# ufcg-lsd/custom-k8s-scheduler

Hardware: AMD Instinct MI355X
Metric: pods scheduled/sec (exact sequential stream, 5,000 nodes x 100,000 pods) (higher is better)
Workload: dtype int32+f64; 1 GPU; config2: 5,000 nodes x 100,000 pods, exact sequential, Fit+Balanced+QoS weights, percentageOfNodesToScore=100; engine=lookahead, launch=resident, table_layout=compact, lookahead=32, parallelism=single

## Files before the change

custom-k8s-scheduler_amd/csrc/qs_ctx.hpp:

```cpp
#pragma once
#include <hip/hip_runtime.h>
#include <rccl/rccl.h>

#include <mutex>
#include <string>
#include <vector>

#include "../../include/qsched.h"
#include "qs_device.hpp"
#include "qs_launch.hpp"

namespace qs_host {

constexpr int64_t kLimit = (1LL << 24) - 1;
constexpr int64_t kWideMemLimit = (1LL << 46) - 1;
constexpr int64_t kGrowLimit32 = (1LL << 31) - 1;
constexpr int64_t kGrowLimitF64 = (1LL << 53) - 1;
constexpr uint32_t kSoaMinNodes = 1u << 16;
constexpr uint32_t kAaMaxNodes = 1u << 20;

struct QsError {
    qs_status st;
    std::string msg;
};

#define HIPCHK(x)                                                                          \
    do {                                                                                   \
        hipError_t e_ = (x);                                                               \
        if (e_ != hipSuccess)                                                              \
            throw QsError{QS_EDEVICE, std::string(#x) + ": " + hipGetErrorString(e_)};     \
    } while (0)

[[noreturn]] inline void fail(qs_status st, const std::string &m) { throw QsError{st, m}; }

inline thread_local std::string g_open_err;
inline qs_status open_failed(qs_status st, const std::string &m) {
    g_open_err = m;
    return st;
}

struct DevBuf {
    void *p = nullptr;
    size_t bytes = 0;
    void ensure(size_t b) {
        if (b <= bytes) return;
        if (p) (void)hipFree(p);
        p = nullptr;
        bytes = 0;
        HIPCHK(hipMalloc(&p, b));
        bytes = b;
    }
    ~DevBuf() {
        if (p) (void)hipFree(p);
    }
    template <class T>
    T *as() const { return (T *)p; }
};

struct Mirror {
    uint32_t n = 0;
    std::vector<int64_t> ac, am, mp, rc, rm, zc, zm, np;
    std::vector<int64_t> ae, re;
    std::vector<uint64_t> th, ts, lb;
    std::vector<int32_t> zone;
    std::vector<uint64_t> gen;
    void resize(uint32_t nn) {
        n = nn;
        zone.assign(nn, 0);
        for (auto *v : {&ac, &am, &mp, &rc, &rm, &zc, &zm, &np}) v->assign(nn, 0);
        ae.assign((size_t)nn * QS_MAX_EXT, 0);
        re.assign((size_t)nn * QS_MAX_EXT, 0);
        th.assign(nn, 0);
        ts.assign(nn, 0);
        lb.assign((size_t)nn * 2, 0);
        gen.assign(nn, 0);
    }
};

inline int ctz64(int64_t v) { return v == 0 ? 64 : __builtin_ctzll((uint64_t)v); }

}

struct qs_stream {
    uint32_t p = 0;
    uint32_t feat = 0;
    std::vector<qs_pod> pods;
    std::vector<uint32_t> order;
    qs_host::DevBuf d_pods, d_podx, d_node, d_key, d_stamp;
    bool ran = false;
    int mode_ran = -1;
    uint64_t epoch_after = 0;
    int shift = 0;
    bool wide = false;
    qs_ctx *owner = nullptr;
    hipGraphExec_t gexec = nullptr;
    std::vector<uint8_t> gkey;
    ~qs_stream() {
        if (gexec) (void)hipGraphExecDestroy(gexec);
    }
};

struct qs_ctx {
    std::mutex mu;
    uint64_t table_epoch = 0;
    qs_config cfg{};
    int device = 0;
    hipStream_t stream = nullptr;
    hipStream_t stream2 = nullptr;
    std::string err;
    qs_host::Mirror m;
    int shift = 20;
    bool wide = false;
    bool dev_valid = false;
    uint32_t zero_alloc = 0;
    qs::DevTable dt{};
    qs::DevCfg dc{};
    qs_scoring_strategy strat[3] = {};
    qs_host::DevBuf strat_tab;
    std::vector<qs_stream *> streams;
    qs_host::DevBuf tbl;
    qs_host::DevBuf soa;
    bool soa_valid = false;
    qs_host::DevBuf tbl_saved;
    qs_host::Mirror m_saved;
    bool saved = false;
    bool saved_wide = false;
    int saved_shift = 20;
    bool mirror_stale = false;
    uint64_t device_faults = 0;
    qs_host::DevBuf diag;
    qs_host::DevBuf scratch, lists, clists, dio, npart, normi, nstat, nfall, nrec, bctrl, one_pod, one_podx;
    qs_host::DevBuf vshard;
    void *pin = nullptr;
    size_t pin_bytes = 0;
    uint64_t score_seq = 0;
    qs_host::DevBuf score_gs;
    uint32_t pend = 0xFFFFFFFFu;
    qs_host::DevBuf hand;
    bool handoff_off = false;
    qs_host::DevBuf resctl;
    int res_timeouts = 0;
    bool res_cooldown = false;
    uint32_t inject_used = 0;
    bool last_resident = false;
    int32_t last_res_path = 0;
    int cus = 0;
    uint64_t run_seq = 0;
    bool last_waits = false;
    uint32_t cap = 0;
    int rank = 0, world = 1;
    ncclComm_t comm = nullptr;
    qs_host::DevBuf mbox, mbox_peers;
    std::vector<void *> mbox_opened;
    bool mbox_on = false;
    bool mbox_fine = false;
    bool mbox_broken = false;
    bool mbox_host = false;
    void *mbox_hptr = nullptr;
    std::string mbox_shm;
    std::vector<void *> mbox_hmaps;
};
namespace qs_host {
void mbox_host_release(qs_ctx *c);
}

namespace qs_host {
struct ShardPlan {
    uint32_t W, v0, nv;
};
inline ShardPlan shard_plan(const qs_ctx *c) {
    if (c->world > 1) return {(uint32_t)c->world, (uint32_t)c->rank, 1u};
    if (c->cfg.virtual_shards > 1) return {(uint32_t)c->cfg.virtual_shards, 0u, (uint32_t)c->cfg.virtual_shards};
    return {1u, 0u, 1u};
}
void exchange_lists(qs_ctx *c, uint64_t *lists, size_t per_rank_entries, hipStream_t stream);
void exchange_u32(qs_ctx *c, uint32_t *buf, size_t per_rank_words, hipStream_t stream);
// ... 26 lines not shown
```

custom-k8s-scheduler_amd/csrc/qs_device.hpp:

```cpp
#pragma once
#include <hip/hip_runtime.h>
#include <hip/hip_fp16.h>
#include <stddef.h>
#include <stdint.h>

#include <type_traits>

namespace qs {

constexpr int kWave = 64;
#define QS_BAL_MAX 4

struct alignas(16) DRow {
    int32_t ac, am;
    int32_t rc, rm;
    int32_t zc, zm;
    int32_t np, mp;
    double yc, ym;
    int32_t ae0, re0, ae1, re1;
};
struct alignas(16) DRowW {
    int32_t rc, zc, np, ac;
    double rm, zm;
    double am, ym;
// ... 251 lines not shown
    constexpr int RB = (int)((F & kFeatWide) ? sizeof(DRowW) : sizeof(DRow));
    constexpr int XQ = (F & kFeatWide) ? 64 : 48;
    const u32x4 a = __builtin_amdgcn_raw_buffer_load_b128(rs, (int)i * RB, 0, 16);
    const u32x4 b = __builtin_amdgcn_raw_buffer_load_b128(rs, (int)i * RB + 16, 0, 16);
    RowT<F> r;
    if constexpr ((F & kFeatWide) != 0) {
        const int4 *q = reinterpret_cast<const int4 *>(t.wrows + i);
        const double2 c = reinterpret_cast<const double2 *>(t.wrows + i)[2];
        const int4 d = q[3];
        r.rc = (int32_t)a.x; r.zc = (int32_t)a.y; r.np = (int32_t)a.z; r.ac = (int32_t)a.w;
        r.rm = u2d(b.x, b.y); r.zm = u2d(b.z, b.w);
        r.am = c.x; r.ym = c.y;
        r.yc = u2d((uint32_t)d.x, (uint32_t)d.y);
        r.mp = d.z;
    } else {
        const double2 y = reinterpret_cast<const double2 *>(t.rows + i)[2];
        r.ac = (int32_t)a.x; r.am = (int32_t)a.y; r.rc = (int32_t)a.z; r.rm = (int32_t)a.w;
        r.zc = (int32_t)b.x; r.zm = (int32_t)b.y; r.np = (int32_t)b.z; r.mp = (int32_t)b.w;
        r.yc = y.x; r.ym = y.y;
    }
    x = RowX{};
    if (F & kFeatExt) {
        const u32x4 e = __builtin_amdgcn_raw_buffer_load_b128(rs, (int)i * RB + XQ, 0, 16);
        x.ae0 = (int32_t)e.x; x.re0 = (int32_t)e.y; x.ae1 = (int32_t)e.z; x.re1 = (int32_t)e.w;
    }
    return r;
}
template <uint32_t F>
__device__ __forceinline__ void store_row_coh(const DevTable &t, __amdgpu_buffer_rsrc_t rs, uint32_t i,
                                              const RowT<F> &r, const RowX &x) {
    (void)t;
    constexpr int RB = (int)((F & kFeatWide) ? sizeof(DRowW) : sizeof(DRow));
    constexpr int XQ = (F & kFeatWide) ? 64 : 48;
    u32x4 a, b;
    if constexpr ((F & kFeatWide) != 0) {
        const uint64_t rm = __builtin_bit_cast(uint64_t, r.rm), zm = __builtin_bit_cast(uint64_t, r.zm);
        a = u32x4{(uint32_t)r.rc, (uint32_t)r.zc, (uint32_t)r.np, (uint32_t)r.ac};
        b = u32x4{(uint32_t)rm, (uint32_t)(rm >> 32), (uint32_t)zm, (uint32_t)(zm >> 32)};
    } else {
        a = u32x4{(uint32_t)r.ac, (uint32_t)r.am, (uint32_t)r.rc, (uint32_t)r.rm};
        b = u32x4{(uint32_t)r.zc, (uint32_t)r.zm, (uint32_t)r.np, (uint32_t)r.mp};
    }
    __builtin_amdgcn_raw_buffer_store_b128(a, rs, (int)i * RB, 0, 16);
    __builtin_amdgcn_raw_buffer_store_b128(b, rs, (int)i * RB + 16, 0, 16);
    if (F & kFeatExt) {
        const u32x4 e = {(uint32_t)x.ae0, (uint32_t)x.re0, (uint32_t)x.ae1, (uint32_t)x.re1};
        __builtin_amdgcn_raw_buffer_store_b128(e, rs, (int)i * RB + XQ, 0, 16);
    }
}

struct RowQ {
    u32x4 a, b, e;
};
template <uint32_t F>
__device__ __forceinline__ RowQ load_row_q(__amdgpu_buffer_rsrc_t rs, uint32_t i) {
    static_assert((F & kFeatWide) == 0, "compact rows only");
    constexpr int kAux = 16 | (int)(1u << 31);
    RowQ q;
    q.a = __builtin_amdgcn_raw_buffer_load_b128(rs, (int)(i * sizeof(DRow)), 0, kAux);
    q.b = __builtin_amdgcn_raw_buffer_load_b128(rs, (int)(i * sizeof(DRow) + 16), 0, kAux);
    q.e = u32x4{0u, 0u, 0u, 0u};
    if (F & kFeatExt) q.e = __builtin_amdgcn_raw_buffer_load_b128(rs, (int)(i * sizeof(DRow) + 48), 0, kAux);
    return q;
}
__device__ __forceinline__ double rcp_int(int32_t a);
template <uint32_t F>
__device__ __forceinline__ Row decode_row_q(const RowQ &q, RowX &x) {
    Row r;
    r.ac = (int32_t)q.a.x; r.am = (int32_t)q.a.y; r.rc = (int32_t)q.a.z; r.rm = (int32_t)q.a.w;
    r.zc = (int32_t)q.b.x; r.zm = (int32_t)q.b.y; r.np = (int32_t)q.b.z; r.mp = (int32_t)q.b.w;
    r.yc = r.ac ? rcp_int(r.ac) : 0.0;
    r.ym = r.am ? rcp_int(r.am) : 0.0;
    x = RowX{};
    if (F & kFeatExt) { x.ae0 = (int32_t)q.e.x; x.re0 = (int32_t)q.e.y; x.ae1 = (int32_t)q.e.z; x.re1 = (int32_t)q.e.w; }
    return r;
}

template <class R, class P>
__device__ __forceinline__ void reserve(R &r, RowX &x, const P &p, int sign) {
    r.rc += sign * p.rc; r.rm += sign * p.rm;
    r.zc += sign * p.zc; r.zm += sign * p.zm;
    r.np += sign;
    x.re0 += sign * p.re0; x.re1 += sign * p.re1;
}

template <uint32_t F, class R, class P>
__device__ __forceinline__ bool fits(const R &r, const RowX &x, const P &p) {
    bool ok = r.np < r.mp;
    ok &= (p.rc <= 0) | (p.rc <= r.ac - r.rc);
    ok &= (p.rm <= 0) | (p.rm <= r.am - r.rm);
    if (F & kFeatExt) {
        ok &= (p.re0 == 0) | (p.re0 <= x.ae0 - x.re0);
        ok &= (p.re1 == 0) | (p.re1 <= x.ae1 - x.re1);
    }
    return ok;
}
__device__ __forceinline__ bool subset128(uint64_t m0, uint64_t m1, uint64_t b0, uint64_t b1) {
    return ((m0 & ~b0) | (m1 & ~b1)) == 0;
}
__device__ __forceinline__ uint64_t uniform64(uint64_t v) {
    const uint32_t lo = (uint32_t)__builtin_amdgcn_readfirstlane((int)(uint32_t)v);
    const uint32_t hi = (uint32_t)__builtin_amdgcn_readfirstlane((int)(uint32_t)(v >> 32));
    return ((uint64_t)hi << 32) | lo;
}
template <uint32_t F, class R, class P>
__device__ __forceinline__ bool feasible(const R &r, const RowX &x, const P &p, const DPodX &px) {
    bool ok = fits<F>(r, x, p);
    if (F & kFeatTaint) ok &= (x.th & ~px.tol_hard) == 0;
    if (F & kFeatAffinity) {
        const uint64_t s0 = uniform64(px.sel0), s1 = uniform64(px.sel1);
        if (s0 | s1) ok &= subset128(s0, s1, x.lb0, x.lb1);
        const uint32_t nt = (uint32_t)__builtin_amdgcn_readfirstlane((int)((p.flags >> 4) & 7u));
        if (nt != 0) {
            bool any = false;
#pragma unroll
            for (uint32_t k = 0; k < 4; ++k)
                if (k < nt) any |= subset128(px.req[k][0], px.req[k][1], x.lb0, x.lb1);
            ok &= any;
        }
    }
    return ok;
}
__device__ __forceinline__ uint32_t taint_raw(const RowX &x, const DPodX &px) {
    return (uint32_t)__popcll(x.ts & ~px.tol_soft);
}
template <class P>
__device__ __forceinline__ uint32_t affinity_raw(const RowX &x, const P &p, const DPodX &px) {
    const uint32_t nt = (uint32_t)__builtin_amdgcn_readfirstlane((int)((p.flags >> 8) & 7u));
    uint32_t s = 0;
#pragma unroll
    for (uint32_t k = 0; k < 4; ++k)
        if (k < nt) s += subset128(px.pref[k][0], px.pref[k][1], x.lb0, x.lb1) ? (uint32_t)px.pw[k] : 0u;
    return s;
}

__device__ __forceinline__ uint32_t static_raw(uint64_t th, uint64_t ts, uint64_t lb0, uint64_t lb1, uint32_t flags,
                                               const DPodX &px) {
    const uint32_t nr = (flags >> 4) & 7u, np = (flags >> 8) & 7u;
    uint32_t ok = (uint32_t)((th & ~px.tol_hard) == 0) & (uint32_t)(((px.sel0 | px.sel1) == 0) | subset128(px.sel0, px.sel1, lb0, lb1));
    uint32_t any = (uint32_t)(nr == 0), ra = 0;
#pragma unroll
    for (uint32_t k = 0; k < 4; ++k) {
        any |= (uint32_t)(k < nr) & (uint32_t)subset128(px.req[k][0], px.req[k][1], lb0, lb1);
        const uint32_t hit = (uint32_t)(k < np) & (uint32_t)subset128(px.pref[k][0], px.pref[k][1], lb0, lb1);
        ra += (0u - hit) & (uint32_t)px.pw[k];
    }
    const uint32_t rt = (uint32_t)__popcll(ts & ~px.tol_soft);
    return (ok & any) | (rt << 1) | (ra << 8);
}

__device__ __forceinline__ uint32_t floor_div(uint32_t n, double y) {
    return (uint32_t)__builtin_fma((double)n, y, 0x1p-30);
}
__device__ __forceinline__ uint32_t least_requested(int32_t a, int32_t reqd, double ya) {
    const int32_t rq = reqd < a ? reqd : a;
    const uint32_t n = __umul24((uint32_t)(a - rq), 100u);
    const uint32_t q = floor_div(n, ya);
    return reqd > a ? 0u : q;
}
__device__ __forceinline__ double fraction(int32_t a, int32_t r, double y) {
    const double R = (double)r, A = (double)a;
    const double q0 = R * y;
    const double rem = __builtin_fma(-q0, A, R);
    const double q = __builtin_fma(rem, y, q0);
    return r >= a ? 1.0 : q;
}
// ... 290 lines not shown
```

custom-k8s-scheduler_amd/csrc/qs_host.cpp:

```cpp
#include "../../include/qsched.h"

#include <hip/hip_runtime.h>

#include <algorithm>
#include <atomic>
#include <chrono>
#include <cmath>
#include <cstddef>
#include <cstdio>
#include <cstdlib>
#include <cstring>
#include <exception>
#include <mutex>
#include <new>
#include <string>
#include <vector>
#include <functional>
#include <condition_variable>
#include <thread>

#include "qs_ctx.hpp"

using namespace qs;

// ... 1233 lines not shown
        std::memset(c->pin, 0, pb);
    }
    if (!c->score_gs.p) {
        c->score_gs.ensure(32);
        HIPCHK(hipMemsetAsync(c->score_gs.p, 0, 32, c->stream));
    }
    const uint32_t pidx = c->pend < n ? c->pend : 0xFFFFFFFFu;
    const HostRow prow = pidx < n ? compact_row(c->m, pidx, c->shift, c->wide) : HostRow{};
    const uint64_t seq = ++c->score_seq;
    const auto tl = std::chrono::steady_clock::now();
    HIPCHK(launch_score_pod1(c->dt, dp, &dx, dc, static_cast<uint8_t *>(c->pin), c->score_gs.as<uint64_t>(), seq,
                             pidx, prow, c->stream));
    c->pend = 0xFFFFFFFFu;
    volatile uint64_t *done = reinterpret_cast<volatile uint64_t *>(static_cast<uint8_t *>(c->pin) + 8);
    const auto t0 = std::chrono::steady_clock::now();
    while (*done != seq) {
        if (std::chrono::steady_clock::now() - t0 > std::chrono::milliseconds(200)) {
            HIPCHK(hipStreamSynchronize(c->stream));
            if (*done != seq) fail(QS_EDEVICE, "qs_score_pod: the scoring kernel did not complete");
            break;
        }
    }
    if (g_sdiag) {
        g_split.tl = tl;
        g_split.t0 = t0;
        g_split.te = std::chrono::steady_clock::now();
    }
    std::atomic_thread_fence(std::memory_order_acquire);
    const uint8_t *h = static_cast<const uint8_t *>(c->pin);
    uint64_t kbest = 0;
    std::memcpy(&kbest, h, 8);
    if (best) *best = kbest ? (int32_t)(0xFFFFFFFFu - (uint32_t)kbest) : -1;
    return reinterpret_cast<const uint32_t *>(h + 16);
}

qs_status qs_score_pod(qs_ctx *c, const qs_pod *pod, uint8_t *feas, int32_t *score, int32_t *total,
                       int32_t *best) {
    return guarded(c, [&] {
        uint32_t w[4];
        const uint32_t *pk = score_pod_launch(c, pod, w, best);
        if (pk) unpack_scores(pk, c->m.n, w, feas, score, total);
        if (g_sdiag && pk) score_diag_report(c->score_seq, std::chrono::steady_clock::now());
    }, true);
}

qs_status qs_score_pod_packed(qs_ctx *c, const qs_pod *pod, const uint32_t **packed, int32_t *best) {
    return guarded(c, [&] {
        uint32_t w[4];
        const uint32_t *pk = score_pod_launch(c, pod, w, best);
        if (packed) *packed = pk;
        if (g_sdiag && pk) score_diag_report(c->score_seq, std::chrono::steady_clock::now());
    }, true);
}

qs_status qs_stream_prepare(qs_ctx *c, const qs_pod *pods, uint32_t p, qs_stream **out) {
    if (!out) return QS_EINVAL;
    *out = nullptr;
    qs_stream *s = nullptr;
    qs_status st = guarded(c, [&] {
        if (p && !pods) fail(QS_EINVAL, "null pods");
        HIPCHK(hipSetDevice(c->device));
        s = new qs_stream();
        s->p = p;
        s->pods.assign(pods, pods + p);
        for (uint32_t j = 0; j < p; j++) check_pod(pods[j], j);
        ensure_layout(c, pods, p);
        s->shift = c->shift;
        s->wide = c->wide;
        s->feat = feat_of(c->cfg) | (c->wide ? kFeatWide | kFeatExt : 0u);
        bool has_ext = false;
        for (uint32_t j = 0; j < p && !has_ext; j++) has_ext = pods[j].req_ext[0] || pods[j].req_ext[1];
        if (has_ext) s->feat |= kFeatExt;
        s->feat |= res_feat(c->cfg, has_ext) | strat_feat(c, pods, p);
        s->order = qos_order(pods, p, c->cfg.qos_sort != 0);
        const size_t rb = pod_record_bytes(c->wide);
        std::vector<uint8_t> dp(rb * std::max<uint32_t>(p, 1));
        const bool needx = feat_of(c->cfg) & (kFeatTaint | kFeatAffinity);
        std::vector<DPodX> dx(needx ? std::max<uint32_t>(p, 1) : 1);
        for (uint32_t k = 0; k < p; k++) {
            const uint32_t j = s->order[k];
            compact_pod(c, pods[j], j, c->shift, c->wide, dp.data() + rb * k);
            if (needx) dx[k] = compact_podx(c, pods[j]);
        }
        const size_t P1 = std::max<uint32_t>(p, 1);
        s->d_pods.ensure(rb * P1);
        s->d_podx.ensure(sizeof(DPodX) * dx.size());
        s->d_node.ensure(4 * P1);
        s->d_key.ensure(8 * P1);
        if (c->cfg.record_timestamps) s->d_stamp.ensure(8 * P1);
        HIPCHK(hipMemcpyAsync(s->d_pods.p, dp.data(), rb * p, hipMemcpyHostToDevice, c->stream));
        HIPCHK(hipMemcpyAsync(s->d_podx.p, dx.data(), sizeof(DPodX) * dx.size(), hipMemcpyHostToDevice, c->stream));
        HIPCHK(hipStreamSynchronize(c->stream));
        c->streams.push_back(s);
        s->owner = c;
    });
    if (st != QS_OK) {
        delete s;
        return st;
    }
    *out = s;
    return QS_OK;
}

qs_status qs_stream_run(qs_ctx *c, qs_stream *s, qs_mode mode, qs_stats *stats) {
    return guarded(c, [&] {
        if (!s) fail(QS_EINVAL, "null stream");
        if (mode != QS_MODE_EXACT && mode != QS_MODE_BATCHED) fail(QS_EINVAL, "unknown qs_mode");
        if (s->shift != c->shift || s->wide != c->wide) fail(QS_ESTATE, "node table re-laid out after prepare");
        HIPCHK(hipSetDevice(c->device));
        s->ran = false;
        s->mode_ran = -1;
        ++c->table_epoch;
        if (!c->dev_valid) upload_table(c);
        const uint32_t n = c->m.n, P = s->p;
        c->dc.feat = s->feat;
        const int eng = mode == QS_MODE_BATCHED ? QS_ENGINE_BATCHED : pick_engine(c, n);
        int32_t *on = s->d_node.as<int32_t>();
        uint64_t *ok = s->d_key.as<uint64_t>();
        uint64_t *st = c->cfg.record_timestamps ? s->d_stamp.as<uint64_t>() : nullptr;
        uint64_t batches = 0;
        hipEvent_t e0, e1;
        HIPCHK(hipEventCreate(&e0));
        HIPCHK(hipEventCreate(&e1));
        KernelTimer kt(c->cfg.profile_kernels != 0, c->stream, c->stream2);
        HIPCHK(hipEventRecord(e0, c->stream));
        if (P > 0 && n == 0) {
            HIPCHK(hipMemsetAsync(on, 0xFF, 4 * (size_t)P, c->stream));
            HIPCHK(hipMemsetAsync(ok, 0, 8 * (size_t)P, c->stream));
        } else if (P > 0) {
            const void *dp = s->d_pods.p;
            const DPodX *dx = s->d_podx.as<DPodX>();
            if (eng == QS_ENGINE_BATCHED) {
                batches = run_batched(c, s, dp, dx, on, ok, kt);
            } else if (eng == QS_ENGINE_PERSISTENT) {
                kt.begin(0, c->stream);
                HIPCHK(launch_persistent(c->dt, dp, dx, P, c->dc, on, ok, st, c->stream));
                kt.end(0, c->stream);
                batches = 1;
            } else if (eng == QS_ENGINE_SCAN) {
                HIPCHK(hipMemsetAsync(c->scratch.p, 0, scan_scratch_bytes(), c->stream));
                ensure_soa(c);
                for (uint32_t k = 0; k < P; k++) {
                    kt.begin(1, c->stream);
                    HIPCHK(launch_scan_pod(c->dt, dp, dx, k, c->dc, c->scratch.p, on, ok, st,
                                           nullptr, nullptr, nullptr, 1, c->stream));
                    kt.end(1, c->stream);
                    HIPCHK(launch_scan_pod(c->dt, dp, dx, k, c->dc, c->scratch.p, on, ok, st,
                                           nullptr, nullptr, nullptr, 2, c->stream));
                }
                batches = P;
            } else if (eng == QS_ENGINE_ALLREDUCE) {
                if (!c->comm)
                    fail(QS_ESTATE, "the all-reduce engine needs an RCCL communicator (qs_open_shard with an id)");
                const uint32_t V = c->world == 1 && c->cfg.virtual_shards > 1 ? (uint32_t)c->cfg.virtual_shards : 1u;
                const uint32_t R = V > 1 ? V : (uint32_t)c->world;
                DevTable dt = c->dt;
                std::memset(&dt.soa, 0, sizeof dt.soa);
                std::vector<uint32_t> sh(2 * (size_t)R);
                for (uint32_t r = 0; r < R; ++r) {
                    sh[2 * r] = (uint32_t)((uint64_t)n * r / R);
                    sh[2 * r + 1] = (uint32_t)((uint64_t)n * (r + 1) / R);
                }
                const uint32_t r0 = V > 1 ? 0u : (uint32_t)c->rank;
                c->vshard.ensure(8 * (size_t)R);
                HIPCHK(hipMemcpy(c->vshard.p, sh.data(), 8 * (size_t)R, hipMemcpyHostToDevice));
                HIPCHK(hipMemsetAsync(c->scratch.p, 0, scan_scratch_bytes(), c->stream));
                char *lohi = static_cast<char *>(c->scratch.p) + offsetof(ScanHead, lo);
                auto range = [&](uint32_t r) {
                    return hipMemcpyAsync(lohi, c->vshard.as<uint32_t>() + 2 * r, 8, hipMemcpyDeviceToDevice, c->stream);
                };
                if (V == 1) HIPCHK(range(r0));
                ScanHead *sc = c->scratch.as<ScanHead>();
                const bool norm = (c->dc.feat & (kFeatTaint | kFeatAffinity)) != 0;
                for (uint32_t k = 0; k < P; k++) {
                    kt.begin(1, c->stream);
                    if (norm) {
                        for (uint32_t v = 0; v < V; ++v) {
                            if (V > 1) HIPCHK(range(v));
                            HIPCHK(launch_scan_pod(dt, dp, dx, k, c->dc, c->scratch.p, on, ok, st, nullptr, nullptr,
                                                   nullptr, 8, c->stream));
                        }
                        allreduce_max_u32(c, &sc->mt, 2, c->stream);
                    }
                    for (uint32_t v = 0; v < V; ++v) {
                        if (V > 1) HIPCHK(range(v));
                        HIPCHK(launch_scan_pod(dt, dp, dx, k, c->dc, c->scratch.p, on, ok, st, nullptr, nullptr,
                                               nullptr, 16 | 32, c->stream));
                    }
                    allreduce_max_u64(c, reinterpret_cast<uint64_t *>(&sc->best), 1, c->stream);
                    HIPCHK(launch_scan_pod(dt, dp, dx, k, c->dc, c->scratch.p, on, ok, st, nullptr, nullptr,
                                           nullptr, 64, c->stream));
                    kt.end(1, c->stream);
                }
                batches = P;
// ... 137 lines not shown
                        }
                    }
                    hipEvent_t eend = nullptr;
                    if (handoff) {
                        HIPCHK(hipEventCreateWithFlags(&eend, hipEventDisableTiming));
                        HIPCHK(hipEventRecord(eend, c->stream2));
                        HIPCHK(hipStreamWaitEvent(c->stream, eend, 0));
                    }
                    for (int r = 0; r < R; ++r) {
                        (void)hipEventDestroy(esel[r]);
                        (void)hipEventDestroy(eres[r]);
                    }
                    (void)hipEventDestroy(est);
                    if (eend) (void)hipEventDestroy(eend);
                }
                };
                static const char *genv = getenv("QS_GRAPH");
                const bool graph_ok = !c->comm || (genv && genv[0] == '1');
                const bool use_graph = graph_ok && !handoff && !mbox && !kt.on && !diag_on && !(genv && genv[0] == '0');
                const char *renv = getenv("QS_RESIDENT");
                if (!c->cus) {
                    int cu = 0;
                    HIPCHK(hipDeviceGetAttribute(&cu, hipDeviceAttributeMultiprocessorCount, c->device));
                    c->cus = cu;
                }
                LaGeom pgeo = geo;
                if (norm && overlap && !(nw && nw[0] == '1')) pgeo.waves = 4;
                const char *rk = getenv("QS_RES_K32");
                if (rk && rk[0] == '0') pgeo.k32 = 0;
                LaGeom rgeo = la_stream_res_plan(pgeo, c->dc.feat, n, (uint32_t)c->cus, 2);
                if (rgeo.G > 0 && rgeo.K * rgeo.G + 1 > la_stream_res_max_blocks(rgeo, c->dc.feat, n, (uint32_t)c->cus))
                    rgeo = la_stream_res_plan(pgeo, c->dc.feat, n, (uint32_t)c->cus, 1);
                static const char *senv = getenv("QS_RES_SEL");
                uint32_t sel = rgeo.K * rgeo.G;
                if (senv && atoi(senv) > 0) sel = (uint32_t)atoi(senv);
                if (norm) sel = std::max(sel, rgeo.K * rgeo.G);
                const bool coresident =
                    rgeo.G > 0 && 1 + sel <= la_stream_res_max_blocks(rgeo, c->dc.feat, n, (uint32_t)c->cus);
                const bool res_transport = c->world == 1 ? !mbox && !c->comm : mbox;
                const bool res_allowed = c->res_timeouts < 2 && !c->res_cooldown;
                const bool resident = overlap && res_transport && res_allowed && !diag_on &&
                                      !(renv && renv[0] == '0') && rgeo.G > 0 && coresident;
                c->last_resident = resident;
                if (!resident) c->res_cooldown = false;
                if (resident) {
                    c->resctl.ensure(la_stream_res_ctl_bytes());
                    c->dc.ready = nullptr;
                    c->dc.epoch = 0;
                    c->dc.werr = reinterpret_cast<uint32_t *>(hw + 2);
                    c->last_waits = true;
                    HIPCHK(hipMemsetAsync(c->lists.p, 0, 8 * lwords * nbuf, c->stream));
                    HIPCHK(hipMemsetAsync(c->dio.p, 0, 2 * kDioWords * 4, c->stream));
                    HIPCHK(hipMemsetAsync(c->resctl.p, 0, la_stream_res_ctl_bytes(), c->stream));
                    HIPCHK(hipMemsetAsync(hw + 2, 0, 8, c->stream));
                    c->npart.ensure(16 * 2 * (size_t)rgeo.K * rgeo.G);
                    c->normi.ensure(16 * 2 * 64);
                    c->nstat.ensure(4 * 2 * 128 * (size_t)rgeo.K);
                    HIPCHK(hipMemsetAsync(c->nfall.p, 0, 16, c->stream));
                    const size_t rcw = std::max<size_t>(1, (size_t)rgeo.K * rgeo.G * rgeo.L);
                    c->clists.ensure(8 * rcw * 2);
                    ResShard rsh{1u, 0u, 0ull, nullptr, 0ull, 0ull, 0ull, 0ull, 0ull};
                    if (c->world > 1)
                        rsh = ResShard{(uint32_t)c->world, (uint32_t)c->rank, seq_run, c->mbox_peers.as<char *>(),
                                       kMbResHello, kMbResFlags, kMbResLists, kMbResNFlags, kMbResNorm};
                    DevCfg dcr = c->dc;
                    const char *inj = getenv("QS_INJECT_FAULT");
                    dcr.inject = (inject_once(c, "resident_stall", kInjResidentStall) ||
                                  (inj && std::strcmp(inj, "resident_stall_always") == 0)) ? 1u : 0u;
                    if (inj && std::strcmp(inj, "resident_skew") == 0) dcr.inject = 2u;
                    dcr.first_ticks = c->world > 1 ? 500000000ull : 0ull;
                    const char *fa = getenv("QS_FAST_ALLOC");
                    dcr.all_alloc = c->zero_alloc == 0 && !(fa && fa[0] == '0') ? 1u : 0u;
                    c->last_res_path = (!norm && rgeo.k32 ? 1 : 0) |
                                       (!norm && !(c->dc.feat & kFeatRes) && dcr.all_alloc ? 2 : 0);
                    static const bool rdiag_on = getenv("QS_RES_DIAG") && (getenv("QS_RES_DIAG")[0] == '1' ||
                                                                             getenv("QS_RES_DIAG")[0] == '2');
                    dcr.sel_diag = getenv("QS_RES_DIAG") && getenv("QS_RES_DIAG")[0] == '1' ? 1u : 0u;
                    uint64_t *rdiag = nullptr;
                    if (rdiag_on) {
                        c->diag.ensure(1024);
                        rdiag = c->diag.as<uint64_t>();
                        HIPCHK(hipMemsetAsync(rdiag, 0, 1024, c->stream));
                    }
                    kt.begin(3, c->stream);
                    HIPCHK(launch_la_stream_res(c->dt, dp, dx, dcr, P, rgeo, L0, c->clists.as<uint64_t>(),
                                                (uint32_t)lwords, (uint32_t)rcw, c->npart.as<uint4>(),
                                                c->normi.as<NormInfo>(), c->nstat.as<uint32_t>(),
                                                c->nfall.as<unsigned long long>(), on, ok,
                                                st, c->resctl.p, sel, rdiag, rsh, c->stream));
                    kt.end(3, c->stream);
                    if (rdiag) {
                        uint64_t h[128] = {0};
                        HIPCHK(hipMemcpyAsync(h, rdiag, 1024, hipMemcpyDeviceToHost, c->stream));
                        HIPCHK(hipStreamSynchronize(c->stream));
                        const double nw = h[3] ? (double)h[3] : 1.0;
                        fprintf(stderr, "QS_RES_DIAG resolver %.3f us per window; windows whose lists were not prefetched %llu of %llu (selectors %u)\n",
                                h[1] * 0.01 / nw, (unsigned long long)h[4], (unsigned long long)h[3], sel);
                        if (h[2])
                            fprintf(stderr, "QS_RES_DIAG selector 0: done seen %.2f us, its task finished %.2f us after "
                                            "the resolver's start of the window it overlaps (%llu windows)\n",
                                    h[13] * 0.01 / (double)h[2], h[14] * 0.01 / (double)h[2], (unsigned long long)h[2]);
                        {
                            std::vector<double> fin;
                            for (uint32_t k = 0; k < std::min(sel, 64u); ++k)
                                if (h[64 + k]) fin.push_back(h[64 + k] * 0.01);
                            std::sort(fin.begin(), fin.end());
                            if (!fin.empty()) {
                                fprintf(stderr, "QS_RES_DIAG selectors' mean finish (us after window start), sorted:");
                                for (double v : fin) fprintf(stderr, " %.1f", v);
                                fprintf(stderr, "\n");
                            }
                        }
                        if (h[36] + h[37] + h[38])
                            fprintf(stderr, "QS_RES_DIAG B3 -> B1 busy (ns per window, without the B1 wait): D %.0f, A %.0f, "
                                            "C %.0f\n", h[38] * 10.0 / nw, h[37] * 10.0 / nw, h[36] * 10.0 / nw);
                        if (h[33])
                            fprintf(stderr, "QS_RES_DIAG last list of a window published %.2f us after the start of "
                                            "the window before it (%llu windows; after 13 us %llu, after 15 us %llu)\n",
                                    h[32] * 0.01 / (double)h[33], (unsigned long long)h[33],
                                    (unsigned long long)h[34], (unsigned long long)h[35]);
                        if (h[6])
                            fprintf(stderr, "QS_RES_DIAG prefetch check: %llu windows short of lists, %.2f lists missing "
                                            "on average\n", (unsigned long long)h[6], (double)h[5] / (double)h[6]);
                        if (h[27] + h[28] + h[29] + h[30] + h[31])
                            fprintf(stderr, "QS_RES_DIAG window boundary (ns per window, wave D): bookkeeping %.0f "
                                            "-> B2 %.0f -> B3 %.0f -> B1 %.0f -> pod 0 decided %.0f\n",
                                    h[27] * 10.0 / nw, h[28] * 10.0 / nw, h[29] * 10.0 / nw, h[30] * 10.0 / nw,
                                    h[31] * 10.0 / nw);
                        if (h[19])
                            fprintf(stderr, "QS_RES_DIAG selector task (us): scoring %.2f chunk top-L %.2f publish/merge %.2f (tasks %llu, merges %llu)\n",
                                    h[16] * 0.01 / (double)h[19], h[17] * 0.01 / (double)h[19], h[18] * 0.01 / (double)h[19],
                                    (unsigned long long)h[19], (unsigned long long)h[20]);
                        if (h[12])
                            fprintf(stderr, "QS_RES_DIAG busy cycles/step: D %.0f A %.0f B %.0f C %.0f (steps %llu)\n",
                                    h[8] / (double)h[12], h[9] / (double)h[12], h[10] / (double)h[12],
                                    h[11] / (double)h[12], (unsigned long long)h[12]);
                        if (h[12])
                            fprintf(stderr, "QS_RES_DIAG step marks: D argmax %.0f | A pub+reads %.0f applied %.0f | C reads %.0f keyC %.0f loads %.0f\n",
                                    h[26] / (double)h[12], h[21] / (double)h[12], h[22] / (double)h[12],
                                    h[23] / (double)h[12], h[24] / (double)h[12], h[25] / (double)h[12]);
                    }
                } else if (use_graph) {
                    std::vector<uint8_t> key;
                    auto put = [&](const void *p, size_t nb) {
                        key.insert(key.end(), (const uint8_t *)p, (const uint8_t *)p + nb);
                    };
                    const void *ptrs[] = {c->dt.rows, c->dt.wrows, c->dt.masks, L0, C0, dio, st, (void *)c->comm, dp, dx,
                                          c->npart.p, c->normi.p, c->nfall.p};
                    put(ptrs, sizeof ptrs);
                    put(&c->dt.n, sizeof c->dt.n);
                    put(&c->dc, sizeof c->dc);
                    put(&geo, sizeof geo);
                    put(&overlap, sizeof overlap);
                    if (!s->gexec || s->gkey != key) {
                        if (s->gexec) (void)hipGraphExecDestroy(s->gexec);
                        s->gexec = nullptr;
                        HIPCHK(hipStreamBeginCapture(c->stream, hipStreamCaptureModeThreadLocal));
                        capturing = true;
                        try {
                            enqueue();
                        } catch (...) {
                            hipGraph_t g = nullptr;
                            (void)hipStreamEndCapture(c->stream, &g);
                            if (g) (void)hipGraphDestroy(g);
                            throw;
                        }
                        hipGraph_t g = nullptr;
                        HIPCHK(hipStreamEndCapture(c->stream, &g));
                        const hipError_t ie = hipGraphInstantiate(&s->gexec, g, nullptr, nullptr, 0);
                        (void)hipGraphDestroy(g);
                        HIPCHK(ie);
                        s->gkey = key;
                    }
                    HIPCHK(hipGraphLaunch(s->gexec, c->stream));
                } else {
                    enqueue();
                }
                batches = nwin;
                if (getenv("QS_HOSTTIME"))
                    fprintf(stderr, "QS_HOSTTIME enqueue %.3f ms for %u windows (overlap %d)\n",
                            std::chrono::duration<double>(std::chrono::steady_clock::now() - th0).count() * 1e3,
                            nwin, (int)overlap);
                if (diag_on) {
                    uint64_t h[16] = {0};
                    HIPCHK(hipMemcpyAsync(h, diag, 128, hipMemcpyDeviceToHost, c->stream));
                    HIPCHK(hipStreamSynchronize(c->stream));
                    const double np = h[5] ? (double)h[5] : 1.0;
                    fprintf(stderr, geo.waves == 1 ? "QS_DIAG resolve cycles/pod: cand %.0f issue %.0f fresh %.0f wmax %.0f commit %.0f (pods %llu, G=%u E=%u epl=%u)\n"
                                                   : "QS_DIAG resolve4 busy cycles/pod: D %.0f A %.0f B %.0f C %.0f (C row wait %.0f) (pods %llu, G=%u E=%u epl=%u)\n",
                            h[0] / np, h[1] / np, h[2] / np, h[3] / np, h[4] / np,
                            (unsigned long long)h[5], geo.G, geo.E, geo.epl);
                    if (geo.waves == 4)
                        fprintf(stderr, "QS_DIAG resolve4 pre-score cycles/pod: A %.0f C %.0f; per window: prologue %.0f epilogue %.0f\n",
                                h[6] / np, h[7] / np, h[8] / (double)nwin, h[9] / (double)nwin);
                }
            }
        }
        HIPCHK(hipEventRecord(e1, c->stream));
// ... 174 lines not shown
        if (s->mode_ran != QS_MODE_EXACT) fail(QS_EINVAL, "FitError diagnosis covers exact streams");
        if (s->epoch_after != c->table_epoch) fail(QS_ESTATE, "the node table changed after the stream's run");
        if (mreq && (!pods || !counts)) fail(QS_EINVAL, "null pods / counts");
        const uint32_t P = s->p;
        for (uint32_t q = 0; q < mreq; q++)
            if (pods[q] >= P) fail(QS_EINVAL, "pod index out of range");
        std::memset(counts, 0, sizeof(uint32_t) * QS_FIT_REASONS * (size_t)mreq);
        if (tcounts) std::memset(tcounts, 0, sizeof(uint32_t) * 64 * (size_t)mreq);
        if (!mreq) return;
        HIPCHK(hipSetDevice(c->device));
        sync_mirror(c);
        std::vector<int32_t> node(P);
        if (P) HIPCHK(hipMemcpy(node.data(), s->d_node.p, 4 * (size_t)P, hipMemcpyDeviceToHost));
        std::vector<std::vector<uint32_t>> want(P);
        std::vector<uint32_t> pos_of(P);
        for (uint32_t k = 0; k < P; k++) pos_of[s->order[k]] = k;
        for (uint32_t q = 0; q < mreq; q++) want[pos_of[pods[q]]].push_back(q);
        Mirror m = c->m;
        for (uint32_t k = 0; k < P; k++)
            if (node[k] >= 0) mirror_reserve(m, (uint32_t)node[k], s->pods[s->order[k]], -1);
        const bool taint = c->cfg.enable_taint != 0, aff = c->cfg.enable_affinity != 0;
        auto subset = [](const uint64_t *mask, const uint64_t *bits) {
            return (mask[0] & ~bits[0]) == 0 && (mask[1] & ~bits[1]) == 0;
        };
        for (uint32_t k = 0; k < P; k++) {
            const qs_pod &p = s->pods[s->order[k]];
            if (node[k] < 0 && !want[k].empty()) {
                uint32_t cnt[QS_FIT_REASONS] = {0};
                uint32_t tcnt[64] = {0};
                const bool any_req = p.req_cpu || p.req_mem || p.req_ext[0] || p.req_ext[1];
                for (uint32_t i = 0; i < m.n; i++) {
                    if (taint && (m.th[i] & ~p.tol_hard) != 0) {
                        ++cnt[QS_FIT_TAINT];
                        ++tcnt[__builtin_ctzll(m.th[i] & ~p.tol_hard)];
                        continue;
                    }
                    if (aff) {
                        const uint64_t *lb = &m.lb[2 * (size_t)i];
                        bool ok = subset(p.sel, lb);
                        if (ok && p.n_req_terms > 0) {
                            bool one = false;
                            for (int t = 0; t < p.n_req_terms; t++) one = one || subset(p.req_terms[t], lb);
                            ok = one;
                        }
                        if (!ok) { ++cnt[QS_FIT_AFFINITY]; continue; }
                    }
                    if (m.np[i] + 1 > m.mp[i]) ++cnt[QS_FIT_TOO_MANY_PODS];
                    if (!any_req) continue;
                    if (p.req_cpu > 0 && p.req_cpu > m.ac[i] - m.rc[i]) ++cnt[QS_FIT_CPU];
                    if (p.req_mem > 0 && p.req_mem > m.am[i] - m.rm[i]) ++cnt[QS_FIT_MEMORY];
                    for (int e = 0; e < QS_MAX_EXT; e++) {
                        const int64_t q = p.req_ext[e];
                        if (q != 0 && q > m.ae[(size_t)i * QS_MAX_EXT + e] - m.re[(size_t)i * QS_MAX_EXT + e])
                            ++cnt[QS_FIT_EXT0 + e];
                    }
                }
                for (uint32_t q : want[k]) {
                    std::memcpy(counts + (size_t)q * QS_FIT_REASONS, cnt, sizeof cnt);
                    if (tcounts) std::memcpy(tcounts + (size_t)q * 64, tcnt, sizeof tcnt);
                }
            }
            if (node[k] >= 0) mirror_reserve(m, (uint32_t)node[k], p, +1);
        }
    });
}

qs_status qs_stream_fit_errors(qs_ctx *c, qs_stream *s, const uint32_t *pods, uint32_t mreq, uint32_t *counts) {
    return fit_errors(c, s, pods, mreq, counts, nullptr);
}

qs_status qs_stream_fit_taints(qs_ctx *c, qs_stream *s, const uint32_t *pods, uint32_t mreq, uint32_t *counts,
                               uint32_t *taint_counts) {
    if (!taint_counts && mreq) return QS_EINVAL;
    return fit_errors(c, s, pods, mreq, counts, taint_counts);
}

qs_status qs_stream_stamps(qs_ctx *c, qs_stream *s, uint64_t *stamps) {
    return guarded(c, [&] {
        if (!s || !s->ran || !s->d_stamp.p) fail(QS_ESTATE, "no timestamps recorded");
        HIPCHK(hipMemcpy(stamps, s->d_stamp.p, 8 * (size_t)s->p, hipMemcpyDeviceToHost));
    });
}

}
```

custom-k8s-scheduler_amd/csrc/qs_kernels.hip:

```cpp
#include "qs_kernels.hpp"

namespace qs {

__global__ __launch_bounds__(256) void k_rows_to_soa(DevTable t) {
    const uint32_t i = blockIdx.x * 256 + threadIdx.x;
    if (i >= t.n) return;
    const DRow r = t.rows[i];
    t.soa.c[kSAc][i] = r.ac; t.soa.c[kSAm][i] = r.am; t.soa.c[kSRc][i] = r.rc; t.soa.c[kSRm][i] = r.rm;
    t.soa.c[kSZc][i] = r.zc; t.soa.c[kSZm][i] = r.zm; t.soa.c[kSNp][i] = r.np; t.soa.c[kSMp][i] = r.mp;
    t.soa.c[kSAe0][i] = r.ae0; t.soa.c[kSRe0][i] = r.re0; t.soa.c[kSAe1][i] = r.ae1; t.soa.c[kSRe1][i] = r.re1;
}

__global__ void k_batch_init(uint32_t *ctrl, uint32_t *bidx, uint32_t P, uint32_t B) {
    const uint32_t nb = min(P, B);
    if (threadIdx.x < nb) bidx[threadIdx.x] = threadIdx.x;
    if (threadIdx.x == 0) { ctrl[0] = nb; ctrl[1] = nb; }
}

hipError_t launch_batch_init(uint32_t *ctrl, uint32_t *bidx, uint32_t P, uint32_t B, hipStream_t stream) {
    hipLaunchKernelGGL(k_batch_init, dim3(1), dim3(64), 0, stream, ctrl, bidx, P, B);
    return hipGetLastError();
}

hipError_t batch_claim_prepare() {
// ... 95 lines not shown
    if (t.wrows) return wide_score_pod1(t, pod, podx, c, hout, gs, seq, pidx, prow, stream);
    switch (feat_class(c.feat)) {
        case 0: return score_pod1_f<0>(t, pod, podx, c, hout, gs, seq, pidx, prow, stream);
        case kFeatExt: return score_pod1_f<kFeatExt>(t, pod, podx, c, hout, gs, seq, pidx, prow, stream);
        default:
            return score_pod1_f<kFeatExt | kFeatTaint | kFeatAffinity>(t, pod, podx, c, hout, gs, seq, pidx, prow, stream);
    }
}

__global__ void k_ready_set(uint64_t *ready, uint64_t value) {
    if (threadIdx.x == 0) __hip_atomic_store(ready, value, __ATOMIC_RELEASE, __HIP_MEMORY_SCOPE_AGENT);
}
hipError_t launch_ready_set(uint64_t *ready, uint64_t value, hipStream_t stream) {
    hipLaunchKernelGGL(k_ready_set, dim3(1), dim3(64), 0, stream, ready, value);
    return hipGetLastError();
}

hipError_t launch_la_window(const DevTable &t, const void *pods, const DPodX *podx, uint32_t s0,
                            uint32_t P, const DevCfg &c, const LaGeom &geo, const LaBufs &bf,
                            int32_t *on, uint64_t *ok, uint64_t *st, uint64_t *diag,
                            hipStream_t stream, int part) {
    if (bf.dprev && geo.waves == 1 && !(c.feat & kFeatNorm)) return hipErrorInvalidValue;
    if ((c.feat & kFeatNorm) && diag && geo.waves != 4) return hipErrorInvalidValue;
    if (c.feat & kFeatStrat)
        return t.wrows ? strat_wide_la_window(t, pods, podx, s0, P, c, geo, bf, on, ok, st, diag, stream, part)
                       : strat_compact_la_window(t, pods, podx, s0, P, c, geo, bf, on, ok, st, diag, stream, part);
    if (c.feat & kFeatRes)
        return t.wrows ? res_wide_la_window(t, pods, podx, s0, P, c, geo, bf, on, ok, st, diag, stream, part)
                       : res_compact_la_window(t, pods, podx, s0, P, c, geo, bf, on, ok, st, diag, stream, part);
    if (t.wrows) return wide_la_window(t, pods, podx, s0, P, c, geo, bf, on, ok, st, diag, stream, part);
    if (c.feat & kFeatNorm)
        return la_window_f<kFeatExt | kFeatTaint | kFeatAffinity>(t, pods, podx, s0, P, c, geo, bf, on, ok, st, diag, stream, part);
    if (c.feat & kFeatExt) return la_window_f<kFeatExt>(t, pods, podx, s0, P, c, geo, bf, on, ok, st, diag, stream, part);
    return la_window_f<0>(t, pods, podx, s0, P, c, geo, bf, on, ok, st, diag, stream, part);
}

LaGeom la_stream_res_plan(const LaGeom &geo, uint32_t feat, uint32_t n, uint32_t cus, uint32_t per_cu) {
    LaGeom r = geo;
    r.G = 0;
    const uint32_t fl = feat & ~(kFeatWide | kFeatRes | kFeatStrat);
    const bool fit = fl == 0 || fl == kFeatExt;
    const bool norm = (feat & kFeatNorm) != 0 && geo.K <= kResNormK;
    const bool shard_ok = geo.W == 1 ? geo.nv == 1 && geo.epl == 1
                                     : geo.nv == 1 && geo.K <= 32 && geo.W * geo.L <= (uint32_t)kResBS;
    if (!((fit || norm) && shard_ok && geo.waves == 4 && geo.L <= 64 && n > 0 && cus > geo.K)) return r;
    n = (n + geo.W - 1) / geo.W;
    const bool two = per_cu >= 2 && fit;
    const uint32_t gmax = std::min(two ? 16u : 8u, ((two ? 2u : 1u) * cus - 1) / geo.K);
    if (gmax == 0) return r;
    constexpr uint32_t bs = kResBS;
    static const uint32_t gwant = getenv("QS_RES_G") ? (uint32_t)std::max(0, atoi(getenv("QS_RES_G"))) : 0u;
    const uint32_t gsmall = std::min((cus - 1) / geo.K, (n + 3 * bs - 1) / (3 * bs));
    const uint32_t G0 = std::min(gmax, std::max({gwant, gsmall, (n + 5 * bs - 1) / (5 * bs)}));
    const uint32_t e_need = ((n + G0 - 1) / G0 + bs - 1) / bs;
    uint32_t E = 0;
    for (uint32_t e : {3u, 5u, 7u, 8u, 16u})
        if (e >= e_need) { E = e; break; }
    if (E == 0) return r;
    const uint32_t G = (n + E * bs - 1) / (E * bs);
    const uint32_t e2 = G * geo.L <= bs ? 1u : 2u;
    if (G * geo.L > e2 * bs || (e2 == 2 && (!two || E == 3))) return r;
    r.e2 = e2;
    r.E = E;
    r.chunk = E * bs;
    r.G = G;
    return r;
}
size_t la_stream_res_ctl_bytes() { return kResCtlBytes; }

uint32_t la_stream_res_max_blocks(const LaGeom &geo, uint32_t feat, uint32_t n, uint32_t cus) {
    const int per = (feat & kFeatStrat) ? ((feat & kFeatWide) ? strat_wide_la_stream_res_per_cu(geo, feat, n)
                                                              : strat_compact_la_stream_res_per_cu(geo, feat, n))
                    : (feat & kFeatRes)   ? ((feat & kFeatWide) ? res_wide_la_stream_res_per_cu(geo, feat, n)
                                                              : res_compact_la_stream_res_per_cu(geo, feat, n))
                    : (feat & kFeatWide)  ? wide_la_stream_res_per_cu(geo, feat, n)
                    : (feat & kFeatNorm)  ? la_stream_res_per_cu<kFeatExt | kFeatTaint | kFeatAffinity>(geo, n)
                    : (feat & kFeatExt) ? la_stream_res_per_cu<kFeatExt>(geo, n)
                                        : la_stream_res_per_cu<0>(geo, n);
    const int sgpr_waves = 800 / (((int)kResSgprMax + 15) / 16 * 16 + 16);
    const int safe = std::min(per, sgpr_waves / (kResBS / 64 / 4));
    return (uint32_t)std::max(0, safe) * cus;
}

hipError_t launch_la_stream_res(const DevTable &t, const void *pods, const DPodX *podx, const DevCfg &c, uint32_t P,
                                const LaGeom &geo, uint64_t *lists0, uint64_t *clists0, uint32_t lwords,
                                uint32_t cwords, uint4 *npart, NormInfo *norm, uint32_t *stat, unsigned long long *nfall,
                                int32_t *on, uint64_t *ok, uint64_t *st, void *ctl, uint32_t sel_blocks, uint64_t *rdiag,
                                const ResShard &rsh, hipStream_t stream) {
    if (geo.G == 0 || (uint64_t)t.n * (t.wrows ? sizeof(DRowW) : sizeof(DRow)) >= (1ull << 31))
        return hipErrorInvalidValue;
    if (c.feat & kFeatStrat)
        return (t.wrows ? strat_wide_la_stream_res : strat_compact_la_stream_res)(
            t, pods, podx, c, P, geo, lists0, clists0, lwords, cwords, npart, norm, stat, nfall, on, ok, st, ctl,
            sel_blocks, rdiag, rsh, stream);
    if (c.feat & kFeatRes)
        return (t.wrows ? res_wide_la_stream_res : res_compact_la_stream_res)(
            t, pods, podx, c, P, geo, lists0, clists0, lwords, cwords, npart, norm, stat, nfall, on, ok, st, ctl,
            sel_blocks, rdiag, rsh, stream);
    if (t.wrows)
        return wide_la_stream_res(t, pods, podx, c, P, geo, lists0, clists0, lwords, cwords, npart, norm, stat, nfall, on,
                                  ok, st, ctl, sel_blocks, rdiag, rsh, stream);
    if (c.feat & kFeatNorm)
        return la_stream_res_f<kFeatExt | kFeatTaint | kFeatAffinity>(t, pods, podx, c, P, geo, lists0, clists0, lwords,
                                                                      cwords, npart, norm, stat, nfall, on, ok, st, ctl,
                                                                      sel_blocks, rdiag, rsh, stream);
    if (c.feat & kFeatExt)
        return la_stream_res_f<kFeatExt>(t, pods, podx, c, P, geo, lists0, clists0, lwords, cwords, npart, norm, stat,
                                         nfall, on, ok, st, ctl, sel_blocks, rdiag, rsh, stream);
    return la_stream_res_f<0>(t, pods, podx, c, P, geo, lists0, clists0, lwords, cwords, npart, norm, stat, nfall, on,
                              ok, st, ctl, sel_blocks, rdiag, rsh, stream);
}

LaGeom la_geometry(uint32_t n, uint32_t K, uint32_t W, uint32_t L) {
    static const uint32_t Es[] = {1, 2, 3, 4, 5, 6, 8, 10, 12, 16};
    static const char *env_e = getenv("QS_LA_E");
    const uint32_t e_target = env_e ? (uint32_t)std::max(1, atoi(env_e)) : 5u;
    LaGeom g{};
    g.K = K;
    g.L = std::max(K, L);
    g.W = std::max(1u, W);
    g.v0 = 0;
    g.nv = g.W;
    if (g.W > 16 || g.L > 64) return g;
    const uint32_t ns = (n + g.W - 1) / g.W;
    const uint32_t gmax = 2048u / g.L;
    const uint32_t target = e_target * 256u;
    uint32_t G = std::max(1u, std::min(gmax, (ns + target - 1) / target));
    const uint32_t per = (ns + G - 1) / G;
    const uint32_t e_need = std::max(1u, (per + 255) / 256);
    uint32_t E = 0;
    for (uint32_t e : Es)
        if (e >= e_need) { E = e; break; }
    if (E == 0) return g;
    g.E = E;
    g.chunk = E * 256;
    G = std::max(1u, (ns + g.chunk - 1) / g.chunk);
    g.eplr = 1;
    g.lr = 0;
    g.epl = 1;
    while (g.epl < g.W) g.epl *= 2;
    g.G = G;
    return g;
}

}
```

custom-k8s-scheduler_amd/csrc/qs_kernels.hpp:

```cpp
#pragma once
#include <algorithm>
#include <cstring>

#include "qs_device.hpp"
#include "qs_launch.hpp"

#ifndef QS_EXP_HOOKS
#define QS_EXP_NORM_AB(norm) (norm)
#define QS_EXP_SLOT_KEY(act, r, q)
#define QS_EXP_CAND_KEY(f, tot, cr, p)
#define QS_EXP_PARK_RETURN()
#endif

#include "qs_key32.hpp"

namespace qs {

constexpr uint32_t kFeatNorm = kFeatTaint | kFeatAffinity;

template <int NPT, int BS, uint32_t F>
__global__ __launch_bounds__(BS) void k_persistent(DevTable t, const PodT<F> *__restrict__ pods,
                                                   const DPodX *__restrict__ podx, uint32_t P,
                                                   DevCfg c, int32_t *__restrict__ out_node,
                                                   uint64_t *__restrict__ out_key,
// ... 2107 lines not shown
                    store_coh_u64(reinterpret_cast<uint64_t *>(no), (uint64_t)nf.mt | ((uint64_t)nf.ct << 32));
                    store_coh_u64(reinterpret_cast<uint64_t *>(no) + 1, (uint64_t)nf.ma | ((uint64_t)nf.ca << 32));
                }
            };
            auto publish = [&]() {
                if (rsh.W > 1) {
                    if (!res_cross_merge(lbuf, L, k, w, rsh, hello_ok, okflag, c.werr, c.first_ticks)) return false;
                }
                uint32_t r0;
                if constexpr (NORM)
                    r0 = res_publish_list_norm(lbuf, L, out, &ctl->rdy[b][0], t, pods, podx, s0 + k, P,
                                               stat0 + ((size_t)b * K + k) * 128);
                else
                    r0 = res_publish_list(lbuf, L, out, &ctl->rdy[b][0]);
                if (rdiag && tid == 0 && w >= 2 && r0 + 1 == (w >> 1) * K + kw) {
                    const uint64_t dt_ = __builtin_amdgcn_s_memrealtime() - wstart_;
                    lastp_ += dt_;
                    ++nlast_;
                    late13_ += dt_ > 1300u;
                    late15_ += dt_ > 1500u;
                }
                return true;
            };
            if (G == 1) {
                put_norm();
                if (!publish()) return;
            } else {
                uint64_t *cl = clists + (size_t)k * G * L;
                if ((uint32_t)tid < L) store_coh_u64(cl + (size_t)g * L + tid, lbuf[tid]);
                drain_stores();
                __syncthreads();
                if (tid == 0) okflag = (res_add(&ctl->ticket[b][k]) + 1) % G == 0 ? 1u : 0u;
                __syncthreads();
                if (okflag) {
                    const uint32_t M = G * L;
                    uint64_t e[E2];
                    uint32_t te[E2];
#pragma unroll
                    for (int j = 0; j < E2; ++j) {
                        const uint32_t pos = (uint32_t)w8 * E2 * kWave + (uint32_t)j * kWave + lane;
                        e[j] = pos < M ? load_coh_u64(cl + pos) : 0ull;
                        te[j] = (uint32_t)(e[j] >> 32);
                    }
                    __syncthreads();
                    block_topl<kResBS, E2>(te, L, lbuf, [&](int j) { return e[j]; });
                    __syncthreads();
                    put_norm();
                    if (!publish()) return;
                    ++nmerge;
                }
            }
            __syncthreads();
            if (rdiag && c.sel_diag) {
                const uint64_t t3 = __builtin_amdgcn_s_memrealtime();
                dsc += ts1 - ts0; dtl += ts2 - ts1; dpm += t3 - ts2; ++ntask;
            }
        }
        if (rdiag && tid == 0 && w >= 2) {
            const uint64_t tp = __builtin_amdgcn_s_memrealtime();
            seen_ += tdone_ - wstart_;
            fin_ += tp - wstart_;
            ++nwt_;
        }
    }
    if (rdiag && sid == 0 && tid == 0) { rdiag[13] = seen_; rdiag[14] = fin_; rdiag[2] = nwt_; }
    if (rdiag && tid == 0 && sid < 64) rdiag[64 + sid] = nwt_ ? fin_ / nwt_ : 0ull;
    if (rdiag && tid == 0 && nlast_) {
        atomicAdd((unsigned long long *)&rdiag[32], (unsigned long long)lastp_);
        atomicAdd((unsigned long long *)&rdiag[33], (unsigned long long)nlast_);
        atomicAdd((unsigned long long *)&rdiag[34], (unsigned long long)late13_);
        atomicAdd((unsigned long long *)&rdiag[35], (unsigned long long)late15_);
    }
    if (rdiag && c.sel_diag && tid == 0) {
        atomicAdd((unsigned long long *)&rdiag[16], (unsigned long long)dsc);
        atomicAdd((unsigned long long *)&rdiag[17], (unsigned long long)dtl);
        atomicAdd((unsigned long long *)&rdiag[18], (unsigned long long)dpm);
        atomicAdd((unsigned long long *)&rdiag[19], (unsigned long long)ntask);
        atomicAdd((unsigned long long *)&rdiag[20], (unsigned long long)nmerge);
    }
}

constexpr uint32_t kResNormK = 32;
constexpr uint32_t kResRing = 4;
constexpr uint32_t kResTStride = 65;
constexpr size_t kResLdsMax = 96 * 1024;
constexpr uint32_t kResSgprMax = 112;
template <uint32_t F>
constexpr size_t res_stream_lds_bytes(uint32_t n, bool k32) {
    const size_t kb = (k32 && (F & kFeatNorm) == 0) ? 4 : 8;
    size_t b = ((((size_t)n + 31) / 32 + 3) & ~(size_t)3) * 4 + 4 * 2 * 64 * kb + 2 * 64 * (sizeof(RowT<F>) + sizeof(int4)) +
               2 * sizeof(ResPub) + 3 * 64 * 4 + 64 * (sizeof(RowT<F>) + sizeof(int4)) + 2 * 64 * sizeof(PodT<F>);
    if ((F & kFeatNorm) == 0)
        b += kResRing * 64 * (kb + sizeof(RowT<F>) + sizeof(int4)) + 16;
    if ((F & kFeatNorm) != 0)
        b += 2 * kResNormK * (sizeof(DPodX) + sizeof(NormInfo) + sizeof(double2)) + 2 * 64 * sizeof(RowX) +
             64 * sizeof(RowX) + 64 * (sizeof(RowT<F>) + sizeof(RowX)) + 2 * 64 * 4 + 64 * 4 + 16 * 4 + 8 * 8 + 16 +
             2 * kResNormK * kResTStride * 4 + 2 * 64 * 4 + 2 * kResNormK * 4 + 64 * sizeof(DMask);
    return b;
}
#ifdef QS_RES_DIAG_BLOCK
constexpr bool kResDiag = true;
#else
constexpr bool kResDiag = false;
#endif
#define QS_RSTAMP_BEGIN() if (kResDiag && rdiag) ts_ = diag_stamp();
#define QS_RSTAMP_END() if (kResDiag && rdiag) busy_ += diag_stamp() - ts_;
#define QS_RSTAMP_MARK(k) if (kResDiag && rdiag) sub_[k] += diag_stamp() - ts_;
template <uint32_t F>
__device__ __forceinline__ uint64_t res_rescan_pass(const DevTable &t, const PodT<F> &p, const DPodX &pxi,
                                                    const uint32_t *dirty, const uint32_t *sidx, const RowT<F> *srow,
                                                    const RowX *sxr, const DMask *smask, uint32_t *red_m,
                                                    uint64_t *red_k, const uint32_t *snd, const DevCfg &cv) {
    __syncthreads();
    const int lane = threadIdx.x & 63;
    const uint32_t wid = (threadIdx.x >> 6) - 4;
    const uint32_t n = t.n, nds = *snd;
    constexpr uint32_t U = 2;
    auto rows_at = [&](uint32_t b0, RowT<F>(&r)[U], RowX(&x)[U]) {
#pragma unroll
        for (uint32_t u = 0; u < U; ++u) {
            const uint32_t idx = b0 + 64 * u < n ? b0 + 64 * u : 0u;
            r[u] = load_row<F>(t, idx);
            x[u] = load_rowx<F>(t, idx);
        }
#pragma unroll
        for (uint32_t u = 0; u < U; ++u) {
            const uint32_t idx = b0 + 64 * u;
            if (idx < n && ((dirty[idx >> 5] >> (idx & 31)) & 1u)) {
                uint32_t j = 0;
                while (j + 1 < nds && sidx[j] != idx) ++j;
                r[u] = srow[j];
                x[u] = sxr[j];
                const DMask m = smask[j];
                x[u].th = m.th; x[u].ts = m.ts; x[u].lb0 = m.lb0; x[u].lb1 = m.lb1;
            }
        }
    };
    uint32_t mt = 0, ma = 0;
    for (uint32_t b0 = wid * 64 * U + lane; b0 < n; b0 += 4 * 64 * U) {
        RowT<F> r[U];
        RowX x[U];
        rows_at(b0, r, x);
#pragma unroll
        for (uint32_t u = 0; u < U; ++u) {
            if (b0 + 64 * u < n && feasible<F>(r[u], x[u], p, pxi)) {
                const uint32_t a = (F & kFeatTaint) ? taint_raw(x[u], pxi) : 0u;
                const uint32_t b2 = (F & kFeatAffinity) ? affinity_raw(x[u], p, pxi) : 0u;
                mt = a > mt ? a : mt;
                ma = b2 > ma ? b2 : ma;
            }
        }
    }
    mt = wave_max_u32(mt);
    ma = wave_max_u32(ma);
    if (lane == 0) { red_m[2 * wid] = mt; red_m[2 * wid + 1] = ma; }
    __syncthreads();
#pragma unroll
    for (uint32_t q = 0; q < 4; ++q) {
        mt = red_m[2 * q] > mt ? red_m[2 * q] : mt;
        ma = red_m[2 * q + 1] > ma ? red_m[2 * q + 1] : ma;
    }
    const double ymt = rcp_exact(mt), yma = rcp_exact(ma);
    uint64_t best = 0;
    for (uint32_t b0 = wid * 64 * U + lane; b0 < n; b0 += 4 * 64 * U) {
        RowT<F> r[U];
        RowX x[U];
        rows_at(b0, r, x);
#pragma unroll
        for (uint32_t u = 0; u < U; ++u) {
            const uint32_t idx = b0 + 64 * u;
            const uint32_t tv = node_total<F>(r[u], x[u], p, pxi, cv, mt, ymt, ma, yma, nullptr);
            const uint64_t key = (idx < n && feasible<F>(r[u], x[u], p, pxi)) ? pack_key(tv + 1, idx) : 0ull;
            best = key > best ? key : best;
        }
    }
    uint64_t ks = wave_max_u64(best);
    if (lane == 0) red_k[wid] = ks;
    __syncthreads();
#pragma unroll
    for (uint32_t q = 0; q < 4; ++q) ks = red_k[q] > ks ? red_k[q] : ks;
    return ks;
}
__device__ __forceinline__ uint64_t res_rescan_wait(const uint64_t *red_k) {
    __syncthreads();
    __syncthreads();
    __syncthreads();
    uint64_t ks = 0;
#pragma unroll
    for (uint32_t q = 0; q < 4; ++q) ks = red_k[q] > ks ? red_k[q] : ks;
    return ks;
}

template <uint32_t F, bool K32>
__device__ __forceinline__ void la_resolve4_stream(uint32_t *lds, const DevTable &t, const PodT<F> *__restrict__ pods,
                                                   const DevCfg &c, uint32_t P, uint32_t K, uint32_t nwin,
                                                   const uint64_t *lists0, uint32_t lwords,
                                                   int32_t *__restrict__ out_node, uint64_t *__restrict__ out_key,
                                                   uint64_t *__restrict__ stamps, ResCtl *ctl, uint64_t *rdiag,
                                                   const DPodX *__restrict__ podx, const NormInfo *norm0,
                                                   const uint32_t *stat0, unsigned long long *nfall) {
    constexpr bool NORM = (F & kFeatNorm) != 0;
    constexpr bool R32 = K32 && !NORM;
    using KT = typename std::conditional<R32, uint32_t, uint64_t>::type;
    const int lane = threadIdx.x & 63;
    const int wv = __builtin_amdgcn_readfirstlane(threadIdx.x >> 6);
    const uint32_t nwords = (t.n + 31) / 32;
    uint32_t *dirty = lds;
    char *base = (char *)(lds + ((nwords + 3) & ~3u));
    KT(*keyA)[64] = (KT(*)[64])base; base += 2 * 64 * sizeof(KT);
    KT(*keyB)[64] = (KT(*)[64])base; base += 2 * 64 * sizeof(KT);
    KT(*keyC)[64] = (KT(*)[64])base; base += 2 * 64 * sizeof(KT);
    KT(*C1)[64] = (KT(*)[64])base; base += 2 * 64 * sizeof(KT);
    auto knode = [](KT k) -> uint32_t {
        if constexpr (R32) return k32_node(k);
        else return key_node(k);
    };
    auto kconv = [](uint64_t e) -> KT {
        if constexpr (R32) return k32_from_key(e);
        else return e;
    };
    (void)knode;
    (void)kconv;
    constexpr bool kFastAllocClass = !NORM && (F & kFeatRes) == 0;
    const bool fast_alloc = kFastAllocClass && c.all_alloc != 0u;
    RowT<F>(*stage)[64] = (RowT<F>(*)[64])base; base += 2 * 64 * sizeof(RowT<F>);
    int4(*stagex)[64] = (int4(*)[64])base; base += 2 * 64 * sizeof(int4);
    ResPub *pub = (ResPub *)base; base += 2 * sizeof(ResPub);
    uint32_t *xrank = (uint32_t *)base; base += 64 * 4;
    uint32_t *xnode = (uint32_t *)base; base += 64 * 4;
    uint32_t *dnode = (uint32_t *)base; base += 64 * 4;
    RowT<F> *carry = (RowT<F> *)base; base += 64 * sizeof(RowT<F>);
    int4 *carryx = (int4 *)base; base += 64 * sizeof(int4);
    PodT<F>(*wpods2)[64] = (PodT<F>(*)[64])base; base += 2 * 64 * sizeof(PodT<F>);
    DPodX(*wpodx2)[kResNormK] = (DPodX(*)[kResNormK])base; base += 2 * kResNormK * sizeof(DPodX);
    NormInfo(*wnorm2)[kResNormK] = (NormInfo(*)[kResNormK])base; base += 2 * kResNormK * sizeof(NormInfo);
    double2(*wrcp2)[kResNormK] = (double2(*)[kResNormK])base; base += 2 * kResNormK * sizeof(double2);
    RowX(*stagexN)[64] = (RowX(*)[64])base; base += 2 * 64 * sizeof(RowX);
    RowX *carryxN = (RowX *)base; base += 64 * sizeof(RowX);
    RowT<F> *srow = (RowT<F> *)base; base += 64 * sizeof(RowT<F>);
    RowX *sxr = (RowX *)base; base += 64 * sizeof(RowX);
    uint32_t(*flagC)[64] = (uint32_t(*)[64])base; base += 2 * 64 * 4;
    uint32_t *sidx = (uint32_t *)base; base += 64 * 4;
    uint32_t *red_m = (uint32_t *)base; base += 16 * 4;
    uint64_t *red_k = (uint64_t *)base; base += 8 * 8;
    uint32_t *snd = (uint32_t *)base; base += 16;
    uint32_t *Tcur = (uint32_t *)base; base += kResNormK * kResTStride * 4;
    uint32_t *Tnext = (uint32_t *)base; base += kResNormK * kResTStride * 4;
    uint32_t(*stS)[64] = (uint32_t(*)[64])base; base += 2 * 64 * 4;
    uint32_t(*nflag2)[kResNormK] = (uint32_t(*)[kResNormK])base; base += 2 * kResNormK * 4;
    DMask *smask = (DMask *)base;
    char *rbase = (char *)(wpodx2);
    KT(*ringE)[64] = (KT(*)[64])rbase; rbase += kResRing * 64 * sizeof(KT);
    RowT<F>(*ringR)[64] = (RowT<F>(*)[64])rbase; rbase += kResRing * 64 * sizeof(RowT<F>);
    int4(*ringX)[64] = (int4(*)[64])rbase; rbase += kResRing * 64 * sizeof(int4);
    uint32_t *late = (uint32_t *)rbase;
    const ResPub none{0, 0xFFFFFFFFu, -1, -1, 0, {0, 0}};
    ResPub32 *pub32 = (ResPub32 *)pub;
    const ResPub32 none32{0u, -1, -1, 0u};
    const DPodX px{};
    DevCfg cv = c;
    asm volatile("" : "+v"(cv.yd_both), "+v"(cv.yd_c), "+v"(cv.yd_m), "+v"(cv.wc), "+v"(cv.wm));
    uint64_t ts_ = 0, busy_ = 0, steps_ = 0, sub_[3] = {0, 0, 0};
    uint64_t bseg_[6] = {0, 0, 0, 0, 0, 0}, bt_ = 0;
    auto bmark = [&](int k) {
        if (rdiag) {
            const uint64_t t_ = __builtin_amdgcn_s_memrealtime();
            if (k >= 0 && bt_) bseg_[k] += t_ - bt_;
            bt_ = t_;
        }
    };
    if (wv < 4) __builtin_amdgcn_s_setprio(3);

    for (uint32_t i = threadIdx.x; i < nwords; i += 256) dirty[i] = 0;
    if (threadIdx.x < min(K, P)) wpods2[0][threadIdx.x] = pods[threadIdx.x];
    if (threadIdx.x == 0) {
        if constexpr (R32) pub32[1] = none32;
        else pub[1] = none;
    }
    if constexpr (!NORM) {
        for (uint32_t j = threadIdx.x; j < kResRing * 64; j += 256) (&ringE[0][0])[j] = 0;
        if (threadIdx.x == 0) *late = 1u;
    }
    if constexpr (NORM) {
        constexpr uint32_t q = sizeof(DPodX) / 16;
        for (uint32_t j = threadIdx.x; j < min(K, P) * q; j += kResBS)
            reinterpret_cast<int4 *>(&wpodx2[0][0])[j] = reinterpret_cast<const int4 *>(podx)[j];
    }
    __syncthreads();

    auto rescan_pass = [&](uint32_t i, uint32_t wb) -> uint64_t {
        return res_rescan_pass<F>(t, wpods2[wb][i], wpodx2[wb][i], dirty, sidx, srow, sxr, smask, red_m, red_k, snd,
                                  cv);
    };

    if (wv == 0) {
        uint32_t nd = 0, didx = 0xFFFFFFFFu;
        uint32_t dlow = 0;
        bool won = false;
        for (uint32_t w = 0; w < nwin; ++w) {
            const uint32_t s0 = w * K, kend = min(K, P - s0);
            const uint32_t knext = w + 1 < nwin ? min(K, P - s0 - K) : 0u;
            uint32_t res_k32 = 0;
            ResPub32 pv32 = none32;
            constexpr int PQ = (int)(sizeof(PodT<F>) / 16);
            static_assert(PQ == 2 || PQ == 3, "pod record of two or three 16-byte quads");
            const int4 *pq = reinterpret_cast<const int4 *>(pods + min(s0 + K + (uint32_t)lane, P - 1));
            const int4 npq0 = pq[0], npq1 = pq[1];
            const int4 npq2 = PQ > 2 ? pq[PQ - 1] : make_int4(0, 0, 0, 0);
            uint64_t res_key = 0, res_stamp = 0;
            ResPub pv = none;
            bool stopped = false;
            if (NORM) __syncthreads();
            if (w > 0) bmark(5);
            __syncthreads();
            if (w > 0) bmark(3);
            if (rdiag && lane == 0) store_coh_u64(&rdiag[15], __builtin_amdgcn_s_memrealtime());
            for (uint32_t i = 0; i < kend; ++i) {
                if constexpr (R32) {
                    QS_RSTAMP_BEGIN()
                    const int par = i & 1, pp = par ^ 1;
                    const uint32_t a = keyA[pp][lane], b = keyB[pp][lane], cl = keyC[pp][lane];
                    const uint32_t e1 = C1[pp][lane];
                    const bool pnew = pv32.k != 0u && pv32.slot < 0;
                    const uint32_t sc = (lane == pv32.slot) ? b : a;
                    uint32_t fk = ((uint32_t)lane < nd && sc) ? (sc | dlow) : 0u;
                    const int srcl = pv32.src >= 0 ? pv32.src : 0;
                    const uint32_t cw = (uint32_t)__builtin_amdgcn_readlane((int)cl, srcl);
                    if (pnew && (uint32_t)lane == pv32.nd_old) fk = cw;
                    const uint32_t cand = (pv32.k != 0u && ((e1 ^ pv32.k) & kK32NodeMask) == 0u) ? 0u : e1;
                    const uint32_t m = wave_max_u32_dpp(fk > cand ? fk : cand);
                    ResPub32 np{m, -1, -1, nd};
                    if (m) {
                        const uint32_t mlow = m & kK32NodeMask;
                        const uint64_t own = __ballot((uint32_t)lane < nd && dlow == mlow);
                        if (own) {
                            np.slot = (int32_t)__builtin_ctzll(own);
                            won |= lane == np.slot;
                        } else {
                            np.src = (int32_t)__builtin_ctzll(__ballot(cand == m));
                            if ((uint32_t)lane == nd) { dlow = mlow; won = true; }
                            ++nd;
                            if (lane == 0) {
                                const uint32_t wn = kK32NodeMask - mlow;
                                __hip_atomic_fetch_or(&dirty[wn >> 5], 1u << (wn & 31), __ATOMIC_RELAXED,
                                                      __HIP_MEMORY_SCOPE_WORKGROUP);
                            }
                        }
                    }
                    pv32 = np;
                    if (lane == 0) write_pub32(&pub32[par], np);
                    if ((uint32_t)lane == i) {
                        res_k32 = m;
                        if (stamps) res_stamp = __builtin_amdgcn_s_memrealtime();
                    }
                    if (i == 0 && w > 0) bmark(4);
                    QS_RSTAMP_MARK(0)
                    QS_RSTAMP_END()
                    __syncthreads();
                } else {
                    QS_RSTAMP_BEGIN()
                    const int par = i & 1, pp = par ^ 1;
                    const uint64_t a = keyA[pp][lane], b = keyB[pp][lane], cl = keyC[pp][lane];
                    const uint64_t e1 = C1[pp][lane];
                    uint32_t fcl = 0;
                    NormInfo nf{0, 0, 0, 0};
                    if (NORM) {
                        fcl = flagC[pp][lane];
                        nf = wnorm2[w & 1][i];
                    }
                    const bool pnew = pv.ks != 0 && pv.slot < 0;
                    uint64_t sc = (lane == pv.slot) ? b : a;
                    uint32_t fl = 0;
                    if (NORM) {
                        fl = (uint32_t)sc & 3u;
                        sc &= ~3ull;
                    }
                    uint64_t fk = ((uint32_t)lane < nd && sc) ? (sc | (uint64_t)(0xFFFFFFFFu - didx)) : 0ull;
                    const int srcl = pv.src >= 0 ? pv.src : 0;
                    const uint64_t cw = ((uint64_t)(uint32_t)__builtin_amdgcn_readlane((int)(cl >> 32), srcl) << 32) |
                                        (uint32_t)__builtin_amdgcn_readlane((int)(uint32_t)cl, srcl);
                    if (pnew && (uint32_t)lane == pv.nd_old) fk = cw;
                    bool unsafe = false;
                    if (NORM) {
                        const uint32_t fc = (uint32_t)__builtin_amdgcn_readlane((int)fcl, srcl);
                        if (pnew && (uint32_t)lane == pv.nd_old) fl = fc;
                        if (F & kFeatTaint)
                            unsafe |= nf.mt > 0 && (uint32_t)__popcll(__ballot((uint32_t)lane < nd && (fl & 1u))) >= nf.ct;
                        if (F & kFeatAffinity)
                            unsafe |= nf.ma > 0 && (uint32_t)__popcll(__ballot((uint32_t)lane < nd && (fl & 2u))) >= nf.ca;
                    }
                    if (NORM && unsafe) {
                        if (lane == 0) pub[par] = ResPub{0, 0xFFFFFFFFu, -2, -1, nd, {0, 0}};
                    } else {
                        const uint64_t cand = (pv.ks != 0 && e1 != 0 && key_node(e1) == pv.w) ? 0ull : e1;
                        const uint64_t best = fk > cand ? fk : cand;
                        uint64_t ks;
                        if (K32) {
                            const uint32_t tv = (uint32_t)(best >> 32);
                            const uint32_t k32 = tv ? (tv << 22) | (0x3FFFFFu - key_node(best)) : 0u;
                            const uint32_t m = wave_max_u32_dpp(k32);
// ... 107 lines not shown
    } else if (wv <= 2) {
        auto role_ab = [&](auto fa) {
        constexpr bool FA = decltype(fa)::value;
        RowT<F> S = empty_row<F>();
        RowX SX{};
        uint32_t nd = 0;
        uint32_t pend = 0;
        const __amdgpu_buffer_rsrc_t rs = row_rsrc<F>(t);
        struct PodN {
            NormInfo nf;
            double2 yr;
        };
        auto slot_key = [&](const RowT<F> &r, const RowX &x, const PodT<F> &q, const PodN &pn, uint32_t st) -> KT {
            const bool act = (uint32_t)lane < nd;
            if constexpr (QS_EXP_NORM_AB(NORM)) {
                const bool f = fits<F>(r, x, q) && (st & 1u) != 0u;
                const uint32_t tot = norm_total<F>(r, x, q, cv, st, pn.nf.mt, pn.yr.x, pn.nf.ma, pn.yr.y);
                uint32_t fl = 0;
                if (act && !f) fl = holder_flags<F>(st, pn.nf.mt, pn.nf.ma);
                return ((act && f) ? ((uint64_t)(tot + 1) << 32) : 0ull) | fl;
            }
            QS_EXP_SLOT_KEY(act, r, q)
            const bool f = feasible<F>(r, x, q, px);
            uint32_t tot;
            if constexpr (NORM) tot = node_total<F>(r, x, q, px, cv, 0, 0.0, 0, 0.0, nullptr);
            else tot = fit_bal_total<F, FA>(r, x, q, cv);
            if constexpr (R32) return (act && f) ? k32_score(tot + 1) : 0u;
            else return (act && f) ? ((uint64_t)(tot + 1) << 32) : 0ull;
        };
        auto rpub = [&](int q) -> ResPub {
            if constexpr (R32) {
                const ResPub32 v = read_pub32(&pub32[q]);
                return ResPub{v.k, 0u, v.slot, v.src, v.nd_old, {0, 0}};
            } else {
                return read_pub(&pub[q]);
            }
        };
        uint32_t snew = 0;
        auto apply = [&](const ResPub &pv, int pp, const PodT<F> &pprev, uint32_t gi) {
            if (pv.ks == 0) return;
            if (pv.slot >= 0) {
                if (lane == pv.slot) reserve(S, SX, pprev, +1);
            } else {
                if ((uint32_t)lane == pv.nd_old) {
                    if constexpr (!NORM) {
                        S = ringR[gi % kResRing][pv.src];
                        if (F & kFeatExt) {
                            const int4 e = ringX[gi % kResRing][pv.src];
                            SX.ae0 = e.x; SX.re0 = e.y; SX.ae1 = e.z; SX.re1 = e.w;
                        }
                    } else {
                        S = stage[pp][pv.src];
                    }
                    if constexpr (NORM) {
                        const int4 e = *reinterpret_cast<const int4 *>(&stagexN[pp][pv.src]);
                        SX.ae0 = e.x; SX.re0 = e.y; SX.ae1 = e.z; SX.re1 = e.w;
                        snew = stS[pp][pv.src];
                    }
                    reserve(S, SX, pprev, +1);
                }
                ++nd;
            }
        };
        auto rescan_ab = [&](uint32_t j, uint32_t wb) {
            if (wv == 1 && (uint32_t)lane < nd) {
                srow[lane] = S;
                *reinterpret_cast<int4 *>(&sxr[lane]) = make_int4(SX.ae0, SX.re0, SX.ae1, SX.re1);
            }
            (void)res_rescan_wait(red_k);
            (void)j;
            (void)wb;
            __syncthreads();
        };
        for (uint32_t w = 0; w < nwin; ++w) {
            const uint32_t s0 = w * K, kend = min(K, P - s0);
            const PodT<F> *wp = wpods2[w & 1];
            auto podn = [&](uint32_t k) -> PodN {
                PodN r{};
                if constexpr (NORM)
                    if (k < kend) r = PodN{wnorm2[w & 1][k], wrcp2[w & 1][k]};
                return r;
            };
            if (NORM) __syncthreads();
            if (wv == 1 && nd > 0)
                keyA[1][lane] = slot_key(S, SX, wp[0], podn(0), NORM ? Tcur[lane] : 0u);
            if (w > 0) bmark(0);
            __syncthreads();
            const uint32_t isig = 0;
            PodT<F> pprev = wp[0], pcur = wp[0];
            PodN pnx = podn(1);
            for (uint32_t i = 0; i < kend; ++i) {
                QS_RSTAMP_BEGIN()
                const int par = i & 1, pp = par ^ 1;
                ResPub pv = rpub(pp);
                const PodT<F> pn1 = wp[i + 1];
                const uint32_t tst = NORM ? Tcur[min(i + 1, kResNormK - 1) * kResTStride + lane] : 0u;
                PodN pnn{};
                if (NORM) pnn = podn(i + 2);
                __builtin_amdgcn_sched_barrier(0);
                if (NORM && i > 0 && pv.slot == -2) {
                    rescan_ab(i - 1, w & 1);
                    pv = rpub(pp);
                }
                const uint32_t nd0 = nd;
                QS_RSTAMP_MARK(0)
                if (i > 0) apply(pv, pp, pprev, s0 + i - 1);
                QS_RSTAMP_MARK(1)
                if (wv == 1 && pend && i == isig) {
                    drain_stores();
                    if (lane == 0) __hip_atomic_store((gu32 *)&ctl->done, pend, __ATOMIC_RELAXED, __HIP_MEMORY_SCOPE_AGENT);
                    pend = 0;
                }
                if (i + 1 < kend) {
                    const PodN pnc = pnx;
                    pnx = pnn;
                    RowT<F> s2 = S;
                    RowX x2s = SX;
                    if (wv == 2) reserve(s2, x2s, pcur, +1);
                    const uint32_t st = (nd != nd0 && (uint32_t)lane == nd0) ? snew : tst;
                    (wv == 1 ? keyA : keyB)[par][lane] = slot_key(s2, x2s, pn1, pnc, st);
                }

                pprev = pcur;
                pcur = pn1;
                QS_RSTAMP_END()
                __syncthreads();
            }
            if (NORM && rpub((kend - 1) & 1).slot == -2) rescan_ab(kend - 1, w & 1);
            apply(rpub((kend - 1) & 1), (kend - 1) & 1, pprev, s0 + kend - 1);
            __syncthreads();
            const uint32_t rk = xrank[lane];
            const bool keep = (uint32_t)lane < nd && rk != 0xFFFFFFFFu;
            if (wv == 1 && keep) {
                store_row_coh<F>(t, rs, xnode[lane], S, SX);
                carry[rk] = S;
                if constexpr (NORM) {
                    const DMask m = smask[lane];
                    carryxN[rk] = RowX{SX.ae0, SX.re0, SX.ae1, SX.re1, m.th, m.ts, m.lb0, m.lb1};
                } else {
                    carryx[rk] = make_int4(SX.ae0, SX.re0, SX.ae1, SX.re1);
                }
            }
            if (wv == 1) pend = w + 1;
            __syncthreads();
            nd = (uint32_t)__popcll(__ballot(keep));
            if ((uint32_t)lane < nd) {
                S = carry[lane];
                if constexpr (NORM) {
                    const RowX o = carryxN[lane];
                    SX = RowX{};
                    SX.ae0 = o.ae0; SX.re0 = o.re0; SX.ae1 = o.ae1; SX.re1 = o.re1;
                    if (wv == 1) smask[lane] = DMask{o.th, o.ts, o.lb0, o.lb1};
                } else {
                    const int4 e = carryx[lane];
                    SX.ae0 = e.x; SX.re0 = e.y; SX.ae1 = e.z; SX.re1 = e.w;
                }
            } else {
                S = empty_row<F>();
                SX = RowX{};
            }
            bmark(-1);
        }
        if (wv == 1 && pend) {
            drain_stores();
            if (lane == 0) __hip_atomic_store((gu32 *)&ctl->done, pend, __ATOMIC_RELAXED, __HIP_MEMORY_SCOPE_AGENT);
        }
        };
        if constexpr (kFastAllocClass) {
            if (fast_alloc) role_ab(std::integral_constant<bool, true>{});
            else role_ab(std::integral_constant<bool, false>{});
        } else {
            role_ab(std::integral_constant<bool, false>{});
        }
    } else if (NORM && wv == 3) {
        uint64_t eX = 0, eY = 0, eZ = 0, c1 = 0;
        uint32_t sA1 = 0, sA2 = 0, sB1 = 0, sB2 = 0;
        RowT<F> r1 = empty_row<F>();
        RowX x1{};
        bool pref = false;
        uint64_t pe0 = 0, pe1 = 0, pe2 = 0;
        uint64_t pn0 = 0, pn1w = 0;
        uint32_t rdyv = 0, nfallback = 0;
        uint64_t cdef_ = 0, cmiss_ = 0;
        auto dirty_bit = [&](uint64_t e) -> bool {
            const uint32_t nidx = e ? key_node(e) : 0u;
            return (dirty[nidx >> 5] >> (nidx & 31)) & 1u;
        };
        auto put_norm = [&](uint32_t wb, uint64_t lo, uint64_t hi) {
            const NormInfo nf{(uint32_t)lo, (uint32_t)(lo >> 32), (uint32_t)hi, (uint32_t)(hi >> 32)};
            wnorm2[wb][lane] = nf;
            wrcp2[wb][lane] = make_double2(rcp_exact(nf.mt), rcp_exact(nf.ma));
        };
        for (uint32_t w = 0; w < nwin; ++w) {
            const uint32_t s0 = w * K, kend = min(K, P - s0);
            const uint64_t *lists = lists0 + (size_t)(w & 1) * lwords;
            const uint32_t *stats = NORM ? stat0 + (size_t)(w & 1) * K * 128 : nullptr;
            const PodT<F> *wp = wpods2[w & 1];
            const bool hasnext = w + 1 < nwin;
            const uint32_t knext = hasnext ? min(K, P - s0 - K) : 0u;
            const uint64_t *listsn = lists0 + (size_t)((w + 1) & 1) * lwords;
            const uint32_t *statsn = NORM ? stat0 + (size_t)((w + 1) & 1) * K * 128 : nullptr;
            const uint32_t tnext = ((w + 1) >> 1) * K + knext;
            auto ent = [&](const uint64_t *l, uint32_t pod, uint32_t kk) -> uint64_t {
                return load_coh_u64(l + (size_t)min(pod, kk - 1) * 64 + lane);
            };
            auto stat_load = [&](uint32_t &d1, uint32_t &d2, const uint32_t *sl, uint32_t pod, uint32_t kk) {
                if constexpr (NORM) {
                    const uint32_t *q = sl + (size_t)min(pod, kk - 1) * 128 + lane;
                    d1 = load_coh_u32(q);
                    d2 = load_coh_u32(q + 64);
                }
            };
            auto rescan_c = [&](uint32_t j) {
// ... 103 lines not shown
                        pref = __builtin_amdgcn_readfirstlane(rdyv) >= tnext;
                        if (rdiag && !pref) {
                            cdef_ += tnext - (uint32_t)__builtin_amdgcn_readfirstlane(rdyv);
                            cmiss_ += 1;
                        }
                        if (pref) {
                            __builtin_amdgcn_fence(__ATOMIC_ACQUIRE, "wavefront");
                            pe0 = ent(listsn, 0, knext);
                            pe1 = ent(listsn, 1, knext);
                            pe2 = ent(listsn, 2, knext);
                            if constexpr (NORM) {
                                const uint64_t *nq =
                                    reinterpret_cast<const uint64_t *>(norm0 + (size_t)((w + 1) & 1) * 64 + lane);
                                pn0 = (uint32_t)lane < knext ? load_coh_u64(nq) : 0ull;
                                pn1w = (uint32_t)lane < knext ? load_coh_u64(nq + 1) : 0ull;
                            }
                        }
                    }
                }
                QS_RSTAMP_END()
                __syncthreads();
            };
            const std::integral_constant<bool, false> plain{};
            const std::integral_constant<bool, true> hooked{};
            const std::integral_constant<int, 0> l1{};
            const std::integral_constant<int, 1> l2{};
            const std::integral_constant<int, 2> l0{};
            const uint32_t ih = pfw ? ((kend - 5) & ~1u) : kend;
            uint32_t i = 0;
            for (; i + 1 < ih; i += 2) {
                step(plain, l2, i, eX, sA1, sA2);
                step(plain, l0, i + 1, eY, sB1, sB2);
            }
            for (; i + 1 < kend; i += 2) {
                step(hooked, l1, i, eX, sA1, sA2);
                step(hooked, l1, i + 1, eY, sB1, sB2);
            }
            if (i < kend) step(hooked, l1, i, eX, sA1, sA2);
            if (NORM && pref && (kend & 1)) {
                const uint32_t t1 = sA1, t2 = sA2;
                sA1 = sB1; sA2 = sB2;
                sB1 = t1; sB2 = t2;
            }
            if (NORM && pub[(kend - 1) & 1].slot == -2) rescan_c(kend - 1);
            if (NORM && pref && (uint32_t)lane < knext) put_norm((w + 1) & 1, pn0, pn1w);
            __syncthreads();
            __syncthreads();
            bmark(-1);
        }
        if (rdiag && lane == 0) { rdiag[4] = nfallback; rdiag[5] = cdef_; rdiag[6] = cmiss_; }
    } else if (!NORM && wv == 3) {
        auto role_c = [&](auto fa) {
        constexpr bool FA = decltype(fa)::value;
        KT c1 = 0;
        uint32_t nfallback = 0;
        auto dirty_bit = [&](KT e) -> bool {
            const uint32_t nidx = e ? knode(e) : 0u;
            return (dirty[nidx >> 5] >> (nidx & 31)) & 1u;
        };
        for (uint32_t w = 0; w < nwin; ++w) {
            const uint32_t s0 = w * K, kend = min(K, P - s0);
            const PodT<F> *wp = wpods2[w & 1];
            if (*late) {
                ++nfallback;
                const uint64_t *lists = lists0 + (size_t)(w & 1) * lwords;
                if (lane == 0) (void)res_wait_ge(&ctl->rdy[w & 1][0], (w >> 1) * K + kend, c.werr, res_bound(c, w));
                __builtin_amdgcn_fence(__ATOMIC_ACQUIRE, "wavefront");
                uint64_t e[3];
#pragma unroll
                for (uint32_t j = 0; j < 3; ++j)
                    e[j] = j < kend ? load_coh_u64(lists + (size_t)j * 64 + lane) : 0ull;
#pragma unroll
                for (uint32_t j = 0; j < 3; ++j) ringE[(s0 + j) % kResRing][lane] = kconv(e[j]);
                const uint32_t n0 = e[0] ? key_node(e[0]) : 0u;
                ringR[s0 % kResRing][lane] = load_row<F>(t, n0);
                if (F & kFeatExt) {
                    const RowX x = load_rowx<F>(t, n0);
                    ringX[s0 % kResRing][lane] = make_int4(x.ae0, x.re0, x.ae1, x.re1);
                }
            }
            const KT e0 = ringE[s0 % kResRing][lane];
            c1 = (e0 != 0 && !dirty_bit(e0)) ? e0 : (KT)0;
            C1[1][lane] = c1;
            if (w > 0) bmark(0);
            __syncthreads();
            PodT<F> pcur = wp[0];
            for (uint32_t i = 0; i < kend; ++i) {
                QS_RSTAMP_BEGIN()
                const uint32_t g = s0 + i;
                const int par = i & 1;
                const KT en = ringE[(g + 1) % kResRing][lane];
                const RowT<F> r1 = ringR[g % kResRing][lane];
                RowX x1{};
                if (F & kFeatExt) {
                    const int4 e = ringX[g % kResRing][lane];
                    x1.ae0 = e.x; x1.re0 = e.y; x1.ae1 = e.z; x1.re1 = e.w;
                }
                const PodT<F> pn1 = wp[i + 1];
                const uint32_t en_node = en ? knode(en) : 0u;
                const uint32_t dword = dirty[en_node >> 5];
                QS_RSTAMP_MARK(0)
                RowT<F> cr = r1;
                RowX crx = x1;
                reserve(cr, crx, pcur, +1);
                const bool f = feasible<F>(cr, crx, pn1, px);
                const uint32_t tot = fit_bal_total<F, FA>(cr, crx, pn1, cv);
                QS_EXP_CAND_KEY(f, tot, cr, pn1)
                QS_RSTAMP_MARK(1)
                if (i + 1 < kend) {
                    if constexpr (R32) keyC[par][lane] = (c1 != 0 && f) ? (k32_score(tot + 1) | (c1 & kK32NodeMask)) : 0u;
                    else keyC[par][lane] = (c1 != 0 && f) ? pack_key(tot + 1, key_node(c1)) : 0ull;
                    const bool dirt = ((dword >> (en_node & 31)) & 1u) != 0;
                    c1 = (en != 0 && !dirt) ? en : (KT)0;
                    C1[par][lane] = c1;
                }
                QS_RSTAMP_MARK(2)
                pcur = pn1;
                QS_RSTAMP_END()
                __syncthreads();
            }
            __syncthreads();
            __syncthreads();
            bmark(-1);
        }
        if (rdiag && lane == 0) { rdiag[4] = nfallback; rdiag[5] = 0; rdiag[6] = 0; }
        };
        if constexpr (kFastAllocClass) {
            if (fast_alloc) role_c(std::integral_constant<bool, true>{});
            else role_c(std::integral_constant<bool, false>{});
        } else {
            role_c(std::integral_constant<bool, false>{});
        }
    } else if (!NORM && wv == 4) {
        uint64_t ein = 0;
        bool skip = true;
        for (uint32_t w = 0; w < nwin; ++w) {
            const uint32_t s0 = w * K, kend = min(K, P - s0);
            const bool hasnext = w + 1 < nwin;
            const uint32_t knext = hasnext ? min(K, P - s0 - K) : 0u;
            const uint64_t *lists = lists0 + (size_t)(w & 1) * lwords;
            const uint64_t *listsn = lists0 + (size_t)((w + 1) & 1) * lwords;
            const uint32_t tnext = ((w + 1) >> 1) * K + knext;
            const bool pfw = hasnext && kend >= 6;
            const uint32_t ic = pfw ? kend - 3 : kend - 1;
            bool lt = hasnext;
            uint32_t rdyv = 0;
            __syncthreads();
            for (uint32_t i = 0; i < kend; ++i) {
                const uint32_t g = s0 + i;
                if (!(skip && i == 0)) ringE[(g + 2) % kResRing][lane] = kconv(ein);
                if (i == ic) {
                    if (pfw) lt = !((uint32_t)__builtin_amdgcn_readfirstlane(rdyv) >= tnext);
                    if (lane == 0) *late = lt ? 1u : 0u;
                }
                uint64_t v = 0;
                if (i + 3 < kend) {
                    v = load_coh_u64(lists + (size_t)(i + 3) * 64 + lane);
                } else if (i >= ic && !lt && hasnext) {
                    const uint32_t j = i + 3 - kend;
                    v = load_coh_u64(listsn + (size_t)min(j, knext - 1) * 64 + lane);
                    v = j < knext ? v : 0ull;
                }
                ein = v;
                if (pfw && i + 4 == kend) rdyv = load_coh_u32(&ctl->rdy[(w + 1) & 1][0]);
                __syncthreads();
            }
            skip = lt;
            __syncthreads();
            __syncthreads();
        }
    } else if (!NORM && wv == 5) {
        for (uint32_t w = 0; w < nwin; ++w) {
            const uint32_t s0 = w * K, kend = min(K, P - s0);
            const bool hasnext = w + 1 < nwin;
            const bool pfw = hasnext && kend >= 6;
            __syncthreads();
            for (uint32_t i = 0; i < kend; ++i) {
                const uint32_t g = s0 + i;
                const bool go = i + 1 < kend || (pfw ? *late == 0u : !hasnext);
                if (go) {
                    const KT e = ringE[(g + 1) % kResRing][lane];
                    const uint32_t nd = e ? knode(e) : 0u;
                    const RowT<F> r = load_row<F>(t, nd);
                    ringR[(g + 1) % kResRing][lane] = r;
                    if (F & kFeatExt) {
                        const RowX x = load_rowx<F>(t, nd);
                        ringX[(g + 1) % kResRing][lane] = make_int4(x.ae0, x.re0, x.ae1, x.re1);
                    }
                }
                __syncthreads();
            }
            __syncthreads();
            __syncthreads();
        }
    } else if constexpr (NORM) {
        constexpr uint32_t q = sizeof(DPodX) / 16;
        const uint32_t pw = (uint32_t)(wv - 4);
        uint32_t ndi = 0;
        for (uint32_t w = 0; w < nwin; ++w) {
            const uint32_t s0 = w * K, kend = min(K, P - s0);
            const uint32_t knext = w + 1 < nwin ? min(K, P - s0 - K) : 0u;
            const uint32_t wb = w & 1, nb = (w + 1) & 1;
            const PodT<F> *wp = wpods2[wb];
            const uint32_t id0 = pw * 64 + lane, id1 = id0 + 256;
            const bool h0 = id0 < knext * q, h1 = id1 < knext * q;
            const int4 *src = reinterpret_cast<const int4 *>(podx + (size_t)s0 + K);
            int4 q0 = make_int4(0, 0, 0, 0), q1 = make_int4(0, 0, 0, 0);
            if (h0) q0 = src[id0];
            if (h1) q1 = src[id1];
            uint32_t nfl = 0;
            if (pw == 0 && (uint32_t)lane < knext) nfl = pods[s0 + K + lane].flags;
            const uint32_t qq = (uint32_t)lane & 31u;
            const bool mycur = wv == 4 && lane < 32;
            DPodX myx{};
            uint32_t myf = 0;
            auto load_mine = [&]() {
                myx = mycur ? wpodx2[wb][qq] : wpodx2[nb][qq];
                myf = mycur ? wp[qq].flags : nflag2[nb][qq];
            };
            auto new_slot = [&](uint32_t j, bool cur) {
                QS_EXP_PARK_RETURN()
                const ResPub pv = read_pub(&pub[j & 1]);
                if (pv.ks == 0 || pv.slot >= 0) return;
                const RowX sx = stagexN[j & 1][pv.src];
                const uint32_t l = pv.nd_old;
                if (lane == 0) smask[l] = DMask{sx.th, sx.ts, sx.lb0, sx.lb1};
                const uint32_t st = static_raw(sx.th, sx.ts, sx.lb0, sx.lb1, myf, myx);
                if (lane < 32) {
                    if (cur && qq >= j + 3 && qq < kend) Tcur[qq * kResTStride + l] = st;
                } else if (qq < knext) {
                    Tnext[qq * kResTStride + l] = st;
                }
            };
            auto inherited = [&](uint32_t j) {
                QS_EXP_PARK_RETURN()
                const uint32_t l = 2 * j + (lane < 32 ? 0u : 1u);
                if (l < ndi && qq < knext) {
                    const RowX sx = carryxN[l];
                    Tnext[qq * kResTStride + l] = static_raw(sx.th, sx.ts, sx.lb0, sx.lb1, myf, myx);
                }
            };
            auto rescan_tail = [&](uint32_t j, uint64_t ks) {
                const uint32_t W = ks ? key_node(ks) : 0u;
                const bool slot = __ballot((uint32_t)lane < *snd && sidx[lane] == W) != 0;
                if (!ks || slot) return;
                const int pj = j & 1;
                const RowT<F> rw = load_row<F>(t, W);
                const RowX xw = load_rowx<F>(t, W);
                uint32_t st2 = 0;
                if (j + 2 < kend) st2 = static_raw(xw.th, xw.ts, xw.lb0, xw.lb1, wp[j + 2].flags, wpodx2[wb][j + 2]);
                if (lane == 0) {
                    stage[pj][0] = rw;
                    stagexN[pj][0] = xw;
                    stS[pj][0] = st2;
                }
                if (j + 1 < kend) {
                    RowT<F> cr = rw;
                    RowX crx = xw;
                    reserve(cr, crx, wp[j], +1);
                    const PodT<F> q1 = wp[j + 1];
                    const DPodX qx = wpodx2[wb][j + 1];
                    const NormInfo nf = wnorm2[wb][j + 1];
                    const double2 yr = wrcp2[wb][j + 1];
                    const bool f = feasible<F>(cr, crx, q1, qx);
                    const uint32_t tot = node_total<F>(cr, crx, q1, qx, cv, nf.mt, yr.x, nf.ma, yr.y, nullptr);
                    uint32_t fl = 0;
                    if (!f) {
                        if (F & kFeatTaint) fl |= taint_raw(crx, qx) == nf.mt ? 1u : 0u;
                        if (F & kFeatAffinity) fl |= affinity_raw(crx, q1, qx) == nf.ma ? 2u : 0u;
                    }
                    if (lane == 0) {
                        keyC[pj][0] = f ? pack_key(tot + 1, W) : 0ull;
                        flagC[pj][0] = fl;
                    }
                }
            };
            __syncthreads();
            __syncthreads();
            for (uint32_t i = 0; i < kend; ++i) {
                if (i == 0) {
                    int4 *dst = reinterpret_cast<int4 *>(&wpodx2[nb][0]);
                    if (h0) dst[id0] = q0;
                    if (h1) dst[id1] = q1;
                    if (pw == 0 && (uint32_t)lane < knext) nflag2[nb][lane] = nfl;
                } else if (wv == 4 || wv == 7) {
                    if (i == 1) load_mine();
                    if (wv == 4) new_slot(i - 1, true);
                    else inherited(i - 1);
                }
                __syncthreads();
                if (pub[i & 1].slot == -2) {
                    const uint64_t ks = rescan_pass(i, wb);
                    if (wv == 4) rescan_tail(i, ks);
                    __syncthreads();
                }
            }
            if ((wv == 4 || wv == 7) && kend == 1) load_mine();
            if (wv == 4) new_slot(kend - 1, false);
            if (wv == 7)
                for (uint32_t j = kend - 1; 2 * j < ndi; ++j) inherited(j);
            __syncthreads();
            for (uint32_t idx = id0; idx < knext * 64; idx += 256) {
                const uint32_t qq = idx >> 6, l = idx & 63u, r = xrank[l];
                if (r != 0xFFFFFFFFu) Tcur[qq * kResTStride + r] = Tnext[qq * kResTStride + l];
            }
            ndi = (uint32_t)__popcll(__ballot(xrank[lane] != 0xFFFFFFFFu));
            __syncthreads();
        }
    }
    if (kResDiag && rdiag && lane == 0 && wv < 4) {
        rdiag[8 + wv] = busy_;
        if (wv == 1) { rdiag[21] = sub_[0]; rdiag[22] = sub_[1]; }
        if (wv == 3) { rdiag[23] = sub_[0]; rdiag[24] = sub_[1]; rdiag[25] = sub_[2]; }
        if (wv == 0) rdiag[26] = sub_[0];
        if (wv == 0) rdiag[12] = steps_;
    }
    if (rdiag && lane == 0 && wv == 0)
        for (int k = 0; k < 5; ++k) rdiag[27 + k] = bseg_[k];
    if (rdiag && lane == 0 && wv == 0) rdiag[38] = bseg_[5];
    if (rdiag && lane == 0 && (wv == 1 || wv == 3)) rdiag[wv == 1 ? 37 : 36] = bseg_[0];
}
#undef QS_RSTAMP_BEGIN
#undef QS_RSTAMP_END

template <uint32_t F, int E, int E2, bool K32>
__global__ __launch_bounds__(kResBS) void k_la_stream_res(DevTable t, const PodT<F> *__restrict__ pods, DevCfg c,
                                                       uint32_t P, uint32_t K, uint32_t G, uint32_t L,
                                                       uint32_t chunk, uint32_t nwin, uint64_t *lists0,
                                                       uint64_t *clists0, uint32_t lwords, uint32_t cwords,
                                                       int32_t *__restrict__ out_node,
                                                       uint64_t *__restrict__ out_key,
                                                       uint64_t *__restrict__ stamps, ResCtl *ctl,
                                                       uint64_t *__restrict__ rdiag, const DPodX *__restrict__ podx,
                                                       uint4 *npart0, NormInfo *norm0, uint32_t *stat0,
                                                       unsigned long long *nfall, ResShard rsh) {
    if (blockIdx.x != 0) {
        res_selector<E, E2, F>(t, pods, c, P, K, G, L, chunk, nwin, lists0, clists0, lwords, cwords, ctl,
                               blockIdx.x - 1, gridDim.x - 1, rdiag, podx, npart0, norm0, stat0, rsh);
        return;
    }
    if (rsh.W > 1 && threadIdx.x == 0)
        for (uint32_t r = 0; r < rsh.W; ++r)
            __hip_atomic_store(reinterpret_cast<uint64_t *>(rsh.peers[r] + rsh.hello) + rsh.rank, rsh.seq,
                               __ATOMIC_RELEASE, __HIP_MEMORY_SCOPE_SYSTEM);
    extern __shared__ __attribute__((aligned(16))) uint32_t lds[];
    if ((F & kFeatNorm) == 0 && threadIdx.x >= 384) {
        __syncthreads();
        for (uint32_t w = 0; w < nwin; ++w)
            for (uint32_t j = 0, nb = min(K, P - w * K) + 3; j < nb; ++j) __syncthreads();
        return;
    }
    const uint64_t t0 = rdiag ? __builtin_amdgcn_s_memrealtime() : 0ull;
    la_resolve4_stream<F, K32>(lds, t, pods, c, P, K, nwin, lists0, lwords, out_node, out_key, stamps, ctl, rdiag,
                               podx, norm0, stat0, nfall);
    if (rdiag && threadIdx.x == 0) { rdiag[1] = __builtin_amdgcn_s_memrealtime() - t0; rdiag[3] = nwin; }
}

static hipError_t res_lds_attr(const void *fn, size_t lds4) {
    if (lds4 <= 64 * 1024) return hipSuccess;
    return hipFuncSetAttribute(fn, hipFuncAttributeMaxDynamicSharedMemorySize, (int)lds4);
}
template <uint32_t F>
static hipError_t la_stream_res_f(const DevTable &t, const void *pods, const DPodX *podx, const DevCfg &c, uint32_t P,
                                  const LaGeom &geo, uint64_t *lists0, uint64_t *clists0, uint32_t lwords,
                                  uint32_t cwords, uint4 *npart0, NormInfo *norm0, uint32_t *stat0,
                                  unsigned long long *nfall, int32_t *on, uint64_t *ok, uint64_t *st, void *ctl,
                                  uint32_t sel_blocks, uint64_t *rdiag, const ResShard &rsh, hipStream_t stream) {
    const uint32_t K = geo.K, G = geo.G, L = geo.L, nwin = (P + K - 1) / K;
    if (rsh.W > 1 && (rsh.W * L > (uint32_t)kResBS || K > 32 || rsh.W > 16 || !rsh.peers))
        return hipErrorInvalidValue;
    const uint32_t E2 = geo.e2;
    if (G * L > E2 * (uint32_t)kResBS || (E2 == 2 && (F & kFeatNorm))) return hipErrorInvalidValue;
    const size_t lds4 = res_stream_lds_bytes<F>(t.n, geo.k32 != 0);
    if (lds4 > kResLdsMax) return hipErrorInvalidValue;
    if ((F & kFeatNorm) && (K > kResNormK || sel_blocks < K * G || !podx || !npart0 || !norm0 || !stat0))
        return hipErrorInvalidValue;
    const dim3 grid(1 + sel_blocks);
    const PodT<F> *pp = (const PodT<F> *)pods;
    ResCtl *rc = (ResCtl *)ctl;
#define QS_RESK(EE, EE2, KK)                                                                                          \
    do {                                                                                                              \
    if (hipError_t ea = res_lds_attr((const void *)k_la_stream_res<F, EE, EE2, KK>, lds4); ea != hipSuccess) return ea; \
    hipLaunchKernelGGL((k_la_stream_res<F, EE, EE2, KK>), grid, dim3(kResBS), lds4, stream, t, pp, c, P, K, G, L,       \
                       geo.chunk, nwin, lists0, clists0, lwords, cwords, on, ok, st, rc, rdiag, podx, npart0, norm0,   \
                       stat0, nfall, rsh);                                                                       \
    } while (0)
#define QS_RESE(EE, EE2) \
    else if (geo.E == EE && E2 == EE2) { if (geo.k32) QS_RESK(EE, EE2, true); else QS_RESK(EE, EE2, false); }
#define QS_RESE2(EE) \
    else if (geo.E == EE && E2 == 2 && (F & kFeatNorm) == 0) { \
        if constexpr ((F & kFeatNorm) == 0) { if (geo.k32) QS_RESK(EE, 2, true); else QS_RESK(EE, 2, false); } }
    if (false) {
    }
    QS_RESE(3, 1) QS_RESE(5, 1) QS_RESE(7, 1) QS_RESE(8, 1) QS_RESE(16, 1)
    QS_RESE2(5) QS_RESE2(7) QS_RESE2(8) QS_RESE2(16)
    else return hipErrorInvalidValue;
#undef QS_RESE
#undef QS_RESE2
#undef QS_RESK
    return hipGetLastError();
}
constexpr size_t kResCtlBytes = sizeof(ResCtl);

template <uint32_t F>
static int la_stream_res_per_cu(const LaGeom &geo, uint32_t n) {
    const size_t lds4 = res_stream_lds_bytes<F>(n, geo.k32 != 0);
    const void *fn = nullptr;
#define QS_RESP(EE, KK) \
    if (geo.E == EE && geo.e2 == 1 && (geo.k32 != 0) == KK) fn = (const void *)k_la_stream_res<F, EE, 1, KK>;
    QS_RESP(3, true) QS_RESP(3, false) QS_RESP(5, true) QS_RESP(5, false) QS_RESP(7, true) QS_RESP(7, false)
    QS_RESP(8, true) QS_RESP(8, false) QS_RESP(16, true) QS_RESP(16, false)
#undef QS_RESP
    if constexpr ((F & kFeatNorm) == 0) {
#define QS_RESP2(EE, KK) \
        if (geo.E == EE && geo.e2 == 2 && (geo.k32 != 0) == KK) fn = (const void *)k_la_stream_res<F, EE, 2, KK>;
        QS_RESP2(5, true) QS_RESP2(5, false) QS_RESP2(7, true) QS_RESP2(7, false) QS_RESP2(8, true) QS_RESP2(8, false) QS_RESP2(16, true) QS_RESP2(16, false)
#undef QS_RESP2
    }
    int per = 0;
    if (!fn || res_lds_attr(fn, lds4) != hipSuccess ||
        hipOccupancyMaxActiveBlocksPerMultiprocessor(&per, fn, kResBS, lds4) != hipSuccess) {
        (void)hipGetLastError();
        return 0;
    }
    return per;
}

#ifdef QS_CLAIM_DIAG
static __device__ uint64_t g_claim_diag[5];
#define CLAIM_STAMP0() uint64_t cds[4] = {0, 0, 0, 0}; uint64_t ctp = diag_stamp();
#define CLAIM_STAMP(q) { const uint64_t t_ = diag_stamp(); cds[q] += t_ - ctp; ctp = t_; }
#else
#define CLAIM_STAMP0()
#define CLAIM_STAMP(q)
#endif
constexpr int kClaimWaves = 16;
constexpr uint32_t kClaimNonEmpty = 1u << 31;
constexpr uint32_t kClaimCarried = 64, kClaimNone = 65;
constexpr uint32_t kClLkey = 0, kClLnode = kClLkey + 64 * 64 * 8, kClLazb = kClLnode + 64 * 64 * 4,
                   kClAz = kClLazb + 64 * 64 * 4, kClPend = kClAz + kMaxApps * kMaxZones / 8, kClSrc = kClPend + 256,
                   kClPod = kClSrc + 256, kClNodes = kClPod + 512;
__host__ __device__ constexpr size_t batch_claim_lds_bytes(uint32_t n) {
    return kClNodes + (((size_t)n + 31) / 32 + 1 + 3) / 4 * 16;
}

template <uint32_t F>
__global__ __launch_bounds__(64 * kClaimWaves) void k_batch_claim(
    DevTable t, const PodT<F> *__restrict__ pods, const uint64_t *__restrict__ lists, uint32_t GLp,
    uint32_t *ctrl, uint32_t *bidx, uint32_t P, uint32_t B, int32_t *__restrict__ out_node,
    uint64_t *__restrict__ out_key) {
    extern __shared__ __attribute__((aligned(16))) uint32_t lds[];
    const int tid = threadIdx.x, lane = tid & 63, wv = tid >> 6;
    CLAIM_STAMP0();
    const uint32_t nwords = (t.n + 31) / 32, sent = nwords * 32;
    uint8_t *lb = reinterpret_cast<uint8_t *>(lds);
    uint64_t *lkey = reinterpret_cast<uint64_t *>(lb + kClLkey);
    uint32_t *lnode = reinterpret_cast<uint32_t *>(lb + kClLnode);
    uint32_t *lazb = reinterpret_cast<uint32_t *>(lb + kClLazb);
    uint32_t *claimed_az = reinterpret_cast<uint32_t *>(lb + kClAz);
    uint32_t *pend = reinterpret_cast<uint32_t *>(lb + kClPend);
    uint32_t *rsrc = reinterpret_cast<uint32_t *>(lb + kClSrc);
    uint32_t *lpod = reinterpret_cast<uint32_t *>(lb + kClPod);
    uint32_t *claimed = reinterpret_cast<uint32_t *>(lb + kClNodes);
    const uint32_t nb = ctrl[0], cursor = ctrl[1];
    for (uint32_t i = tid; i < nwords; i += 64 * kClaimWaves) claimed[i] = 0;
    if (tid == 0) claimed[nwords] = 0xFFFFFFFFu;
    for (uint32_t i = tid; i < kMaxApps * kMaxZones / 32; i += 64 * kClaimWaves) claimed_az[i] = 0;
    {
        constexpr int Q = 64 / kClaimWaves;
        uint64_t ev[Q];
        uint32_t fv[Q];
#pragma unroll
        for (int q = 0; q < Q; ++q) {
            const uint32_t i = (uint32_t)wv + kClaimWaves * q;
            ev[q] = i < nb ? lists[(size_t)i * GLp + lane] : 0ull;
            fv[q] = i < nb ? bidx[i] : 0u;
        }
        uint32_t sv[Q];
#pragma unroll
        for (int q = 0; q < Q; ++q) {
            sv[q] = fv[q];
            fv[q] = (uint32_t)wv + kClaimWaves * q < nb ? pods[sv[q]].flags : 0u;
        }
        uint32_t zv[Q];
#pragma unroll
        for (int q = 0; q < Q; ++q)
            zv[q] = (ev[q] && pod_aa(fv[q]) == 2u) ? (uint32_t)t.zone[key_node(ev[q])] : 0u;
#pragma unroll
        for (int q = 0; q < Q; ++q) {
            const uint32_t i = (uint32_t)wv + kClaimWaves * q;
            const bool ok = ev[q] != 0ull;
            lkey[i * 64 + lane] = ev[q];
            lnode[i * 64 + lane] = ok ? key_node(ev[q]) : sent;
            lazb[i * 64 + lane] = pod_app(fv[q]) * kMaxZones + (zv[q] & (kMaxZones - 1));
            const uint32_t ne = __ballot(ok) ? kClaimNonEmpty : 0u;
            if (lane == 0) { lpod[i] = sv[q]; lpod[64 + i] = fv[q] | ne; }
        }
    }
    __syncthreads();
    if (wv != 0) return;
    CLAIM_STAMP(0);
    uint32_t npend = 0;
    const uint32_t my_s = (uint32_t)lane < nb ? lpod[lane] : 0u;
    const uint32_t my_flags = lpod[64 + lane];
    CLAIM_STAMP(1);
    struct Ents {
// ... 380 lines not shown
```

custom-k8s-scheduler_amd/csrc/qs_launch.hpp:

```cpp
#pragma once
#include <hip/hip_runtime.h>
#include <stddef.h>
#include <stdint.h>

namespace qs {

struct DevTable;
struct DevCfg;
struct DPodX;

struct HostRow {
    int32_t ac, am, rc, rm, zc, zm, np, mp;
    double yc, ym;
    int32_t ae0, re0, ae1, re1;
    uint64_t th, ts, lb0, lb1;
    int32_t zone, pad;
    double wam, wrm, wzm;
};

struct LaGeom {
    uint32_t K, L, G, E, chunk, epl, waves, k32;
    uint32_t W, v0, nv, eplr, lr;
    uint32_t e2 = 1;
};
struct LaShard {
    uint32_t W, v0, kw, pad;
    uint64_t RS;
};

hipError_t launch_persistent(const DevTable &t, const void *pods, const DPodX *podx, uint32_t P,
                             const DevCfg &c, int32_t *out_node, uint64_t *out_key,
                             uint64_t *stamps, hipStream_t stream);
uint32_t persistent_max_nodes(uint32_t feat);

hipError_t launch_scan_pod(const DevTable &t, const void *pods, const DPodX *podx, uint32_t s,
                           const DevCfg &c, void *scratch, int32_t *out_node, uint64_t *out_key,
                           uint64_t *stamps, uint8_t *feas, int32_t *score, int32_t *total,
                           int part, hipStream_t stream);
hipError_t launch_rows_to_soa(const DevTable &t, hipStream_t stream);
uint32_t score_pod1_max_nodes();
constexpr uint32_t kScoreInfeasible = 0xFFFFFFFFu;
size_t score_pod1_pack_bytes(uint32_t n);
hipError_t launch_score_pod1(const DevTable &t, const void *pod, const DPodX *podx, const DevCfg &c, uint8_t *hout,
                             uint64_t *gs, uint64_t seq, uint32_t pidx, const HostRow &prow, hipStream_t stream);
size_t scan_scratch_bytes();
struct ScanHead {
    unsigned long long best;
    uint32_t mt, ma, lo, hi;
};

LaGeom la_geometry(uint32_t n, uint32_t K, uint32_t W = 1, uint32_t L = 0);
struct NormInfo;
struct LaBufs {
    uint64_t *lists, *clists;
    uint4 *npart;
    NormInfo *norm;
    const uint32_t *dprev;
    uint32_t *dcur;
    unsigned long long *nfall;
    const uint32_t *pidx = nullptr, *pcount = nullptr;
    uint32_t *rec = nullptr;
    uint32_t *tickets = nullptr;
};
hipError_t launch_ready_set(uint64_t *ready, uint64_t value, hipStream_t stream);

LaGeom la_stream_res_plan(const LaGeom &geo, uint32_t feat, uint32_t n, uint32_t cus, uint32_t per_cu = 1);
size_t la_stream_res_ctl_bytes();
uint32_t la_stream_res_max_blocks(const LaGeom &geo, uint32_t feat, uint32_t n, uint32_t cus);
struct ResShard {
    uint32_t W, rank;
    uint64_t seq;
    char *const *peers;
    uint64_t hello, flags, lists;
    uint64_t nflags, norm;
};
hipError_t launch_la_stream_res(const DevTable &t, const void *pods, const DPodX *podx, const DevCfg &c, uint32_t P,
                                const LaGeom &geo, uint64_t *lists0, uint64_t *clists0, uint32_t lwords,
                                uint32_t cwords, uint4 *npart, NormInfo *norm, uint32_t *stat, unsigned long long *nfall, int32_t *on,
                                uint64_t *ok, uint64_t *st, void *ctl, uint32_t sel_blocks, uint64_t *rdiag,
                                const ResShard &rsh, hipStream_t stream);

hipError_t launch_la_window(const DevTable &t, const void *pods, const DPodX *podx, uint32_t s0,
                            uint32_t P, const DevCfg &c, const LaGeom &geo, const LaBufs &bufs,
                            int32_t *out_node, uint64_t *out_key, uint64_t *stamps, uint64_t *diag,
                            hipStream_t stream, int part);

hipError_t launch_batch_init(uint32_t *ctrl, uint32_t *bidx, uint32_t P, uint32_t B, hipStream_t stream);
size_t batch_claim_lds(uint32_t n);
hipError_t batch_claim_prepare();
hipError_t launch_batch_claim(const DevTable &t, const void *pods, const uint64_t *lists, uint32_t *ctrl,
                              uint32_t *bidx, uint32_t P, uint32_t B, int32_t *out_node,
                              uint64_t *out_key, hipStream_t stream);

__global__ void k_set_row(DevTable t, uint32_t i, HostRow v, uint32_t feat);

}
```

custom-k8s-scheduler_amd/qsched/__init__.py:

```python
from __future__ import annotations

import ctypes

import numpy as np

from ._abi import (ENGINES, ENGINE_NAMES, EXPORTED, LIB_PATH, POD_DTYPE, QS_ABI_VERSION,
                   QS_MAX_EXT, QS_MAX_SCORE_RES, QS_MAX_TERMS, QS_MODE_BATCHED, QS_MODE_EXACT, QS_OK,
                   RESOURCES, FIT_REASONS, QS_FIT_TAINT, QS_MAX_SHAPE, QOS_NAMES, STRATEGIES, QschedError,
                   QschedLibraryMissing, QsConfig, QsContainer, QsNodeRow, QsNodeSoa, QsScoringStrategy,
                   QsStats, load)

__all__ = ["Scheduler", "Config", "POD_DTYPE", "pods_to_struct", "pods_from_struct", "fit_error_message",
           "synth_generate", "shape_table", "dist_unique_id", "empty_nodes", "pod_from_containers", "compute_qos", "load",
           "QschedError", "QschedLibraryMissing", "ENGINES", "EXPORTED", "LIB_PATH"]

MODES = {"exact": QS_MODE_EXACT, "batched": QS_MODE_BATCHED}
NODE_I64 = ["alloc_cpu", "alloc_mem", "max_pods", "req_cpu", "req_mem", "nz_cpu", "nz_mem", "pods"]


def _check(lib, ctx, st):
    if st != QS_OK:
        msg = lib.qs_last_error(ctx).decode() if ctx else ""
        raise QschedError(st, msg)

# ... 177 lines not shown
        self._chk(self.lib.qs_nodes_read(self.ctx, ctypes.byref(s), self.n))
        return out

    def upsert(self, idx, row: dict, generation=0):
        r = QsNodeRow()
        for f, t in QsNodeRow._fields_:
            if f in row:
                v = row[f]
                if f in ("alloc_ext", "req_ext", "label_bits"):
                    for i, x in enumerate(v):
                        getattr(r, f)[i] = int(x)
                else:
                    setattr(r, f, int(v))
        self._chk(self.lib.qs_node_upsert(self.ctx, idx, ctypes.byref(r), generation))
        if idx == self.n:
            self.n += 1

    def save_table(self):
        self._chk(self.lib.qs_table_save(self.ctx))

    def restore_table(self):
        self._chk(self.lib.qs_table_restore(self.ctx))

    def reserve(self, node, pod):
        p = pods_to_struct(pod) if not isinstance(pod, np.void) else np.array([pod], POD_DTYPE)
        self._chk(self.lib.qs_reserve(self.ctx, node, _ptr(p)))

    def unreserve(self, node, pod):
        p = pods_to_struct(pod) if not isinstance(pod, np.void) else np.array([pod], POD_DTYPE)
        self._chk(self.lib.qs_unreserve(self.ctx, node, _ptr(p)))

    def score_pod(self, pod, outputs=True, out=None):
        p = np.array([pod], POD_DTYPE) if isinstance(pod, np.void) else pods_to_struct(pod)[:1]
        best = ctypes.c_int32(-2)
        if not outputs:
            self._chk(self.lib.qs_score_pod(self.ctx, _ptr(p), None, None, None, ctypes.byref(best)))
            return dict(best=best.value)
        if out is None:
            out = self.score_buffers()
        feas, score, total = out["feasible"], out["scores"], out["total"]
        if len(total) != self.n or score.shape != (self.n, 4) or feas.dtype != np.bool_:
            raise ValueError("score_pod: out buffers do not match the node table (use score_buffers())")
        self._chk(self.lib.qs_score_pod(self.ctx, _ptr(p), _ptr(feas), _ptr(score), _ptr(total),
                                        ctypes.byref(best)))
        return dict(feasible=feas, scores=score, total=total, best=best.value)

    def score_pod_packed(self, pod):
        p = np.array([pod], POD_DTYPE) if isinstance(pod, np.void) else pods_to_struct(pod)[:1]
        best = ctypes.c_int32(-2)
        ptr = ctypes.POINTER(ctypes.c_uint32)()
        self._chk(self.lib.qs_score_pod_packed(self.ctx, _ptr(p), ctypes.byref(ptr), ctypes.byref(best)))
        packed = np.ctypeslib.as_array(ptr, shape=(self.n,)).copy() if self.n and ptr else np.zeros(0, np.uint32)
        return best.value, packed

    def score_buffers(self):
        return dict(feasible=np.zeros(self.n, np.bool_), scores=np.zeros((self.n, 4), np.int32),
                    total=np.zeros(self.n, np.int32))

    def schedule(self, pods, with_stats=False, mode="exact"):
        arr = pods_to_struct(pods)
        placement = np.empty(len(arr), np.int32)
        stats = QsStats()
        self._chk(self.lib.qs_schedule_stream(self.ctx, _ptr(arr), len(arr), MODES[mode],
                                              _ptr(placement), ctypes.byref(stats)))
        return (placement, stats.as_dict()) if with_stats else placement

    def prepare(self, pods):
        arr = pods_to_struct(pods)
        h = ctypes.c_void_p()
        self._chk(self.lib.qs_stream_prepare(self.ctx, _ptr(arr), len(arr), ctypes.byref(h)))
        return Stream(self, h, len(arr))


class Stream:

    def __init__(self, sched: Scheduler, handle, p):
        self.s, self.h, self.p = sched, handle, p
        self.stats = None

    def run(self, mode="exact"):
        st = QsStats()
        self.s._chk(self.s.lib.qs_stream_run(self.s.ctx, self.h, MODES[mode], ctypes.byref(st)))
        self.stats = st.as_dict()
        return self.stats

    def results(self):
        placement = np.empty(self.p, np.int32)
        keys = np.empty(self.p, np.uint64)
        self.s._chk(self.s.lib.qs_stream_results(self.s.ctx, self.h, _ptr(placement), _ptr(keys)))
        return placement, keys

    def stamps(self):
        out = np.empty(self.p, np.uint64)
        self.s._chk(self.s.lib.qs_stream_stamps(self.s.ctx, self.h, _ptr(out)))
        return out

    def fit_errors(self, pods=None, by_taint=False):
        if pods is None:
            pl, _ = self.results()
            pods = np.nonzero(pl < 0)[0]
        idx = np.ascontiguousarray(pods, dtype=np.uint32)
        counts = np.zeros((len(idx), len(FIT_REASONS)), np.uint32)
        if not by_taint:
            self.s._chk(self.s.lib.qs_stream_fit_errors(self.s.ctx, self.h, _ptr(idx), len(idx), _ptr(counts)))
            return idx, counts
        tcounts = np.zeros((len(idx), 64), np.uint32)
        self.s._chk(self.s.lib.qs_stream_fit_taints(self.s.ctx, self.h, _ptr(idx), len(idx), _ptr(counts),
                                                     _ptr(tcounts)))
        return idx, counts, tcounts

    def free(self):
        if self.h:
            self.s._chk(self.s.lib.qs_stream_free(self.s.ctx, self.h))
            self.h = None


def dist_unique_id() -> bytes:
    lib = load()
    buf = (ctypes.c_uint8 * 128)()
    st = lib.qs_dist_unique_id(buf)
    if st != QS_OK:
        raise QschedError(st, "qs_dist_unique_id failed")
    return bytes(buf)


def shape_table(shape):
    lib = load()
    shape = list(shape)
    pts = ((ctypes.c_int32 * 2) * max(1, len(shape)))()
    for i, (u, sc) in enumerate(shape):
        pts[i][0], pts[i][1] = int(u), int(sc)
    out = np.zeros(101, np.uint8)
    st = lib.qs_shape_table(pts, len(shape), _ptr(out))
    if st != QS_OK:
        raise QschedError(st, "qs_shape_table: bad shape")
    return out


def synth_generate(config: int, n: int, p: int, seed=None):
    lib = load()
    nodes = empty_nodes(n)
    s, _ = _soa(nodes, lib_out=True)
    pods = np.zeros(p, POD_DTYPE)
    seed = 0x5EED0000 + config if seed is None else seed
    st = lib.qs_synth_generate(config, seed, n, p, ctypes.byref(s), _ptr(pods))
    if st != QS_OK:
        raise QschedError(st, "qs_synth_generate failed")
    return nodes, pods


def _containers(containers):
    arr = (QsContainer * max(1, len(containers)))()
    for i, c in enumerate(containers):
        for k, v in c.items():
            if k == "req_ext":
                for e, x in enumerate(v):
                    arr[i].req_ext[e] = int(x)
            elif k == "kind":
                arr[i].kind = {"regular": 0, "init": 1, "sidecar": 2}.get(v, v)
            elif k in ("req_cpu", "req_mem", "lim_cpu", "lim_mem"):
                setattr(arr[i], k, int(v))
                setattr(arr[i], "has_" + k, 1)
    return arr


def fit_error_message(counts, n_nodes, ext_names=("ext0", "ext1"), taint_counts=None, taint_names=None):
# ... 35 lines not shown
```

custom-k8s-scheduler_amd/qsched/_abi.py:

```python
from __future__ import annotations

import ctypes
import os

import numpy as np

PKG_ROOT = os.path.dirname(os.path.dirname(os.path.abspath(__file__)))
LIB_PATH = os.environ.get("QSCHED_LIB") or os.path.join(PKG_ROOT, "libqsched.so")

QS_ABI_VERSION = 3
QS_MAX_EXT = 2
QS_MAX_TERMS = 4
QS_MAX_APPS = 1024
QS_MAX_ZONES = 64
QS_AA_NONE, QS_AA_HOSTNAME, QS_AA_ZONE = 0, 1, 2
QS_MAX_SCORE_RES = 4
FIT_REASONS = ["Too many pods", "Insufficient cpu", "Insufficient memory", "Insufficient {ext0}",
               "Insufficient {ext1}", "node(s) had untolerated taint {{{taint}}}",
               "node(s) didn't match Pod's node affinity/selector"]
QS_FIT_TAINT = 5
RESOURCES = {"cpu": 1, "memory": 2, "ext0": 3, "ext1": 4}

STRATEGIES = {"LeastAllocated": 0, "MostAllocated": 1, "RequestedToCapacityRatio": 2}
QOS_NAMES = {"BestEffort": 0, "Burstable": 1, "Guaranteed": 2}
# ... 50 lines not shown


class QsNodeRow(ctypes.Structure):
    _fields_ = [("alloc_cpu", ctypes.c_int64), ("alloc_mem", ctypes.c_int64),
                ("alloc_ext", ctypes.c_int64 * QS_MAX_EXT), ("max_pods", ctypes.c_int64),
                ("req_cpu", ctypes.c_int64), ("req_mem", ctypes.c_int64),
                ("req_ext", ctypes.c_int64 * QS_MAX_EXT), ("nz_cpu", ctypes.c_int64),
                ("nz_mem", ctypes.c_int64), ("pods", ctypes.c_int64),
                ("taint_hard", ctypes.c_uint64), ("taint_soft", ctypes.c_uint64),
                ("label_bits", ctypes.c_uint64 * 2), ("zone", ctypes.c_int32),
                ("reserved", ctypes.c_int32)]


class QsContainer(ctypes.Structure):
    _fields_ = [("kind", ctypes.c_int32), ("has_req_cpu", ctypes.c_int32),
                ("has_req_mem", ctypes.c_int32), ("has_lim_cpu", ctypes.c_int32),
                ("has_lim_mem", ctypes.c_int32), ("req_cpu", ctypes.c_int64),
                ("req_mem", ctypes.c_int64), ("lim_cpu", ctypes.c_int64),
                ("lim_mem", ctypes.c_int64), ("req_ext", ctypes.c_int64 * QS_MAX_EXT)]


class QsStats(ctypes.Structure):
    _fields_ = [("pods", ctypes.c_uint64), ("placed", ctypes.c_uint64),
                ("unschedulable", ctypes.c_uint64), ("evals", ctypes.c_uint64),
                ("batches", ctypes.c_uint64), ("truncations", ctypes.c_uint64),
                ("wall_s", ctypes.c_double), ("h2d_s", ctypes.c_double), ("d2h_s", ctypes.c_double),
                ("p50_cycle_us", ctypes.c_double), ("p99_cycle_us", ctypes.c_double),
                ("max_cycle_us", ctypes.c_double), ("engine_used", ctypes.c_int32),
                ("table_layout", ctypes.c_int32), ("resumed_windows", ctypes.c_uint64),
                ("device_faults", ctypes.c_uint64),
                ("resident", ctypes.c_int32), ("resident_path", ctypes.c_int32), ("kernel_s", ctypes.c_double * 4),
                ("kernel_launches", ctypes.c_uint64 * 4)]

    KERNELS = ("persistent", "scan", "select", "resolve")

    def as_dict(self):
        d = {f: getattr(self, f) for f, _ in self._fields_
             if f not in ("reserved", "kernel_s", "kernel_launches")}
        d["engine_used"] = ENGINE_NAMES.get(self.engine_used, self.engine_used)
        d["table_layout"] = LAYOUT_NAMES.get(self.table_layout, self.table_layout)
        d["kernels"] = {k: {"s": self.kernel_s[i], "launches": int(self.kernel_launches[i])}
                        for i, k in enumerate(self.KERNELS) if self.kernel_launches[i]}
        return d


POD_DTYPE = np.dtype([
    ("req_cpu", "<i8"), ("req_mem", "<i8"), ("req_ext", "<i8", (QS_MAX_EXT,)),
    ("nz_cpu", "<i8"), ("nz_mem", "<i8"), ("qos", "<i4"), ("priority", "<i4"),
    ("tol_hard", "<u8"), ("tol_soft", "<u8"), ("sel", "<u8", (2,)),
    ("n_req_terms", "<i4"), ("n_pref_terms", "<i4"),
    ("req_terms", "<u8", (QS_MAX_TERMS, 2)), ("pref_terms", "<u8", (QS_MAX_TERMS, 2)),
    ("pref_weight", "<i4", (QS_MAX_TERMS,)), ("app", "<i4"), ("anti_affinity", "<i4"),
], align=True)

_P = ctypes.c_void_p
_SIGS = {
    "qs_config_default": (None, [_P]),
    "qs_open": (ctypes.c_int, [_P, ctypes.c_int, _P]),
    "qs_open_shard": (ctypes.c_int, [_P, ctypes.c_int, ctypes.c_int, ctypes.c_int, _P, _P]),
    "qs_dist_unique_id": (ctypes.c_int, [_P]),
    "qs_dist_mailbox_export": (ctypes.c_int, [_P, _P]),
    "qs_dist_mailbox_connect": (ctypes.c_int, [_P, _P]),
    "qs_set_scoring_strategy": (ctypes.c_int, [_P, _P]),
    "qs_set_scoring_strategy_qos": (ctypes.c_int, [_P, ctypes.c_int32, _P]),
    "qs_get_scoring_strategy_qos": (ctypes.c_int, [_P, ctypes.c_int32, _P]),
    "qs_shape_table": (ctypes.c_int, [_P, ctypes.c_uint32, _P]),
    "qs_close": (ctypes.c_int, [_P]),
    "qs_last_error": (ctypes.c_char_p, [_P]),
    "qs_version": (ctypes.c_char_p, []),
    "qs_nodes_load": (ctypes.c_int, [_P, _P, ctypes.c_uint32]),
    "qs_nodes_read": (ctypes.c_int, [_P, _P, ctypes.c_uint32]),
    "qs_node_upsert": (ctypes.c_int, [_P, ctypes.c_uint32, _P, ctypes.c_uint64]),
    "qs_table_save": (ctypes.c_int, [_P]),
    "qs_table_restore": (ctypes.c_int, [_P]),
    "qs_reserve": (ctypes.c_int, [_P, ctypes.c_uint32, _P]),
    "qs_unreserve": (ctypes.c_int, [_P, ctypes.c_uint32, _P]),
    "qs_score_pod": (ctypes.c_int, [_P, _P, _P, _P, _P, _P]),
    "qs_score_pod_packed": (ctypes.c_int, [_P, _P, _P, _P]),
    "qs_schedule_stream": (ctypes.c_int, [_P, _P, ctypes.c_uint32, ctypes.c_int, _P, _P]),
    "qs_stream_prepare": (ctypes.c_int, [_P, _P, ctypes.c_uint32, _P]),
    "qs_stream_run": (ctypes.c_int, [_P, _P, ctypes.c_int, _P]),
    "qs_stream_results": (ctypes.c_int, [_P, _P, _P, _P]),
    "qs_stream_stamps": (ctypes.c_int, [_P, _P, _P]),
    "qs_stream_fit_errors": (ctypes.c_int, [_P, _P, _P, ctypes.c_uint32, _P]),
    "qs_stream_fit_taints": (ctypes.c_int, [_P, _P, _P, ctypes.c_uint32, _P, _P]),
    "qs_stream_free": (ctypes.c_int, [_P, _P]),
    "qs_pod_from_containers": (ctypes.c_int, [_P, ctypes.c_uint32, _P, _P]),
    "qs_compute_qos": (ctypes.c_int32, [_P, ctypes.c_uint32]),
    "qs_synth_generate": (ctypes.c_int, [ctypes.c_int, ctypes.c_uint64, ctypes.c_uint32,
                                         ctypes.c_uint32, _P, _P]),
    "qs_struct_size": (ctypes.c_size_t, [ctypes.c_int]),
}
EXPORTED = sorted(_SIGS)

_LIB = None


def load(path: str = LIB_PATH):
    global _LIB
    if _LIB is not None:
        return _LIB
    if not os.path.exists(path):
        raise QschedLibraryMissing(
            f"{path} not found: build it with `make -C custom-k8s-scheduler_amd` (hipcc, gfx950)")
    lib = ctypes.CDLL(path)
    for name, (res, args) in _SIGS.items():
        fn = getattr(lib, name)
        fn.restype = res
        fn.argtypes = args
    expect = {0: ctypes.sizeof(QsConfig), 1: ctypes.sizeof(QsNodeSoa), 2: ctypes.sizeof(QsNodeRow),
              3: POD_DTYPE.itemsize, 4: ctypes.sizeof(QsContainer), 5: ctypes.sizeof(QsStats),
              6: ctypes.sizeof(QsScoringStrategy)}
    for k, v in expect.items():
        got = lib.qs_struct_size(k)
        if got != v:
            raise RuntimeError(f"ABI struct {k} size mismatch: C {got} vs Python {v}")
    _LIB = lib
    return lib
```

include/qsched.h:

```cpp
#ifndef QSCHED_H
#define QSCHED_H

#include <stddef.h>
#include <stdint.h>

#ifdef __cplusplus
extern "C" {
#endif

#if defined(__GNUC__)
#define QS_API __attribute__((visibility("default")))
#else
#define QS_API
#endif

#define QS_ABI_VERSION 3
#define QS_MAX_EXT 2
#define QS_MAX_TERMS 4
#define QS_MAX_APPS 1024
#define QS_MAX_ZONES 64
#define QS_MAX_SCORE_RES 4

typedef enum qs_status {
    QS_OK = 0,
// ... 83 lines not shown

typedef struct qs_node_row {
    int64_t alloc_cpu, alloc_mem, alloc_ext[QS_MAX_EXT], max_pods;
    int64_t req_cpu, req_mem, req_ext[QS_MAX_EXT], nz_cpu, nz_mem, pods;
    uint64_t taint_hard, taint_soft, label_bits[2];
    int32_t zone, reserved;
} qs_node_row;

typedef struct qs_pod {
    int64_t req_cpu, req_mem, req_ext[QS_MAX_EXT];
    int64_t nz_cpu, nz_mem;
    int32_t qos;
    int32_t priority;
    uint64_t tol_hard;
    uint64_t tol_soft;
    uint64_t sel[2];
    int32_t n_req_terms, n_pref_terms;
    uint64_t req_terms[QS_MAX_TERMS][2];
    uint64_t pref_terms[QS_MAX_TERMS][2];
    int32_t pref_weight[QS_MAX_TERMS];
    int32_t app;
    int32_t anti_affinity;
} qs_pod;

typedef struct qs_container {
    int32_t kind;
    int32_t has_req_cpu, has_req_mem, has_lim_cpu, has_lim_mem;
    int64_t req_cpu, req_mem, lim_cpu, lim_mem;
    int64_t req_ext[QS_MAX_EXT];
} qs_container;

typedef struct qs_stats {
    uint64_t pods, placed, unschedulable, evals;
    uint64_t batches, truncations;
    double wall_s;
    double h2d_s, d2h_s;
    double p50_cycle_us, p99_cycle_us, max_cycle_us;
    int32_t engine_used;
    int32_t table_layout;
    uint64_t resumed_windows;
    uint64_t device_faults;
    int32_t resident;
    int32_t resident_path;
    double kernel_s[4];
    uint64_t kernel_launches[4];
} qs_stats;

typedef struct qs_ctx qs_ctx;
typedef struct qs_stream qs_stream;

QS_API void qs_config_default(qs_config *cfg);
QS_API qs_status qs_open(const qs_config *cfg, int device, qs_ctx **out);
QS_API qs_status qs_open_shard(const qs_config *cfg, int device, int rank, int world,
                        const uint8_t nccl_id[128], qs_ctx **out);
QS_API qs_status qs_dist_unique_id(uint8_t out[128]);
QS_API qs_status qs_dist_mailbox_export(qs_ctx *ctx, uint8_t handle[64]);
QS_API qs_status qs_dist_mailbox_connect(qs_ctx *ctx, const uint8_t *handles );
QS_API qs_status qs_set_scoring_strategy(qs_ctx *ctx, const qs_scoring_strategy *s);
QS_API qs_status qs_set_scoring_strategy_qos(qs_ctx *ctx, int32_t qos, const qs_scoring_strategy *s);
QS_API qs_status qs_get_scoring_strategy_qos(qs_ctx *ctx, int32_t qos, qs_scoring_strategy *out);
QS_API qs_status qs_close(qs_ctx *ctx);
QS_API const char *qs_last_error(const qs_ctx *ctx);
QS_API const char *qs_version(void);

QS_API qs_status qs_nodes_load(qs_ctx *ctx, const qs_node_soa *nodes, uint32_t n);
QS_API qs_status qs_nodes_read(qs_ctx *ctx, const qs_node_soa_out *out, uint32_t n);
QS_API qs_status qs_node_upsert(qs_ctx *ctx, uint32_t idx, const qs_node_row *row, uint64_t generation);
QS_API qs_status qs_table_save(qs_ctx *ctx);
QS_API qs_status qs_table_restore(qs_ctx *ctx);
QS_API qs_status qs_reserve(qs_ctx *ctx, uint32_t node, const qs_pod *pod);
QS_API qs_status qs_unreserve(qs_ctx *ctx, uint32_t node, const qs_pod *pod);

QS_API qs_status qs_score_pod(qs_ctx *ctx, const qs_pod *pod, uint8_t *feasible_n, int32_t *score_n,
                       int32_t *total_n, int32_t *best);
QS_API qs_status qs_score_pod_packed(qs_ctx *ctx, const qs_pod *pod, const uint32_t **packed_n, int32_t *best);

QS_API qs_status qs_schedule_stream(qs_ctx *ctx, const qs_pod *pods, uint32_t p, qs_mode mode,
                             int32_t *placement_p, qs_stats *stats);
QS_API qs_status qs_stream_prepare(qs_ctx *ctx, const qs_pod *pods, uint32_t p, qs_stream **out);
QS_API qs_status qs_stream_run(qs_ctx *ctx, qs_stream *s, qs_mode mode, qs_stats *stats);
QS_API qs_status qs_stream_results(qs_ctx *ctx, qs_stream *s, int32_t *placement_p, uint64_t *best_key_p);
QS_API qs_status qs_stream_free(qs_ctx *ctx, qs_stream *s);
QS_API qs_status qs_stream_stamps(qs_ctx *ctx, qs_stream *s, uint64_t *stamps_p);
typedef enum qs_fit_reason {
    QS_FIT_TOO_MANY_PODS = 0,
    QS_FIT_CPU = 1,
    QS_FIT_MEMORY = 2,
    QS_FIT_EXT0 = 3,
    QS_FIT_EXT1 = 4,
    QS_FIT_TAINT = 5,
    QS_FIT_AFFINITY = 6,
    QS_FIT_REASONS = 7
} qs_fit_reason;
QS_API qs_status qs_stream_fit_errors(qs_ctx *ctx, qs_stream *s, const uint32_t *pods, uint32_t m, uint32_t *counts);
QS_API qs_status qs_stream_fit_taints(qs_ctx *ctx, qs_stream *s, const uint32_t *pods, uint32_t m, uint32_t *counts,
                                      uint32_t *taint_counts);

QS_API qs_status qs_pod_from_containers(const qs_container *c, uint32_t nc, const int64_t *overhead_cpu_mem,
                                 qs_pod *out);
QS_API int32_t qs_compute_qos(const qs_container *c, uint32_t nc);
QS_API size_t qs_struct_size(int which);
QS_API qs_status qs_shape_table(const qs_shape_point *shape, uint32_t n, uint8_t table[101]);
QS_API qs_status qs_synth_generate(int config, uint64_t seed, uint32_t n, uint32_t p,
                            const qs_node_soa_out *nodes, qs_pod *pods);

#ifdef __cplusplus
}
#endif
#endif
```

Before: 2.215 million pods/s.

## Add uniform-window fast path to resident stream resolver for identical-pod runs

When every pod in a lookahead window is byte-identical to the one before it, the resident resolver switches to a ladder-based merge. Helper waves precompute per-node score rungs for up to UR successive reservations of the same pod, and one wave then pops the best rung per placement instead of re-scoring each pod sequentially. The host detects such windows from a run-start array and uploads a per-window bitmask, and the kernel gets a UNI template variant. This aims to cut the per-pod resolve and barrier cost in repetitive streams, at the price of more code paths, extra LDS use, and possibly lower occupancy.

```diff
diff --git a/custom-k8s-scheduler_amd/csrc/qs_ctx.hpp b/custom-k8s-scheduler_amd/csrc/qs_ctx.hpp
--- a/custom-k8s-scheduler_amd/csrc/qs_ctx.hpp
+++ b/custom-k8s-scheduler_amd/csrc/qs_ctx.hpp
@@ -92,6 +92,10 @@
     uint64_t epoch_after = 0;
     int shift = 0;
     bool wide = false;
+    std::vector<uint32_t> run0;
+    std::vector<uint32_t> uni_bits;
+    qs_host::DevBuf d_uni;
+    uint32_t uni_K = 0, uni_count = 0, uni_given = 0;
     qs_ctx *owner = nullptr;
     hipGraphExec_t gexec = nullptr;
     std::vector<uint8_t> gkey;
diff --git a/custom-k8s-scheduler_amd/csrc/qs_device.hpp b/custom-k8s-scheduler_amd/csrc/qs_device.hpp
--- a/custom-k8s-scheduler_amd/csrc/qs_device.hpp
+++ b/custom-k8s-scheduler_amd/csrc/qs_device.hpp
@@ -357,6 +357,13 @@
     r.zc += sign * p.zc; r.zm += sign * p.zm;
     r.np += sign;
     x.re0 += sign * p.re0; x.re1 += sign * p.re1;
+}
+template <class R, class P>
+__device__ __forceinline__ void reserve_n(R &r, RowX &x, const P &p, int k) {
+    r.rc += k * p.rc; r.rm += k * p.rm;
+    r.zc += k * p.zc; r.zm += k * p.zm;
+    r.np += k;
+    x.re0 += k * p.re0; x.re1 += k * p.re1;
 }
 
 template <uint32_t F, class R, class P>
diff --git a/custom-k8s-scheduler_amd/csrc/qs_host.cpp b/custom-k8s-scheduler_amd/csrc/qs_host.cpp
--- a/custom-k8s-scheduler_amd/csrc/qs_host.cpp
+++ b/custom-k8s-scheduler_amd/csrc/qs_host.cpp
@@ -1339,6 +1339,9 @@
             compact_pod(c, pods[j], j, c->shift, c->wide, dp.data() + rb * k);
             if (needx) dx[k] = compact_podx(c, pods[j]);
         }
+        s->run0.resize(p);
+        for (uint32_t k = 0; k < p; k++)
+            s->run0[k] = k > 0 && std::memcmp(dp.data() + rb * k, dp.data() + rb * (k - 1), rb) == 0 ? s->run0[k - 1] : k;
         const size_t P1 = std::max<uint32_t>(p, 1);
         s->d_pods.ensure(rb * P1);
         s->d_podx.ensure(sizeof(DPodX) * dx.size());
@@ -1367,6 +1370,7 @@
         HIPCHK(hipSetDevice(c->device));
         s->ran = false;
         s->mode_ran = -1;
+        s->uni_given = 0;
         ++c->table_epoch;
         if (!c->dev_valid) upload_table(c);
         const uint32_t n = c->m.n, P = s->p;
@@ -1670,12 +1674,38 @@
                         rdiag = c->diag.as<uint64_t>();
                         HIPCHK(hipMemsetAsync(rdiag, 0, 1024, c->stream));
                     }
+                    const char *ue = getenv("QS_RES_UNIFORM");
+                    const uint32_t *uni = nullptr;
+                    s->uni_given = 0;
+                    if (!(ue && ue[0] == '0') && la_stream_res_takes_uniform(rgeo, c->dc.feat, rsh.W) &&
+                        s->run0.size() == P) {
+                        if (s->uni_K != rgeo.K) {
+                            const uint32_t K = rgeo.K, nwin = (P + K - 1) / K;
+                            s->uni_bits.assign((nwin + 31) / 32 + 1, 0u);
+                            s->uni_count = 0;
+                            for (uint32_t w = 0; w < nwin; ++w) {
+                                const uint32_t s0 = w * K, last = std::min(P, s0 + K) - 1;
+                                if (s->run0[last] <= s0) {
+                                    s->uni_bits[w >> 5] |= 1u << (w & 31);
+                                    ++s->uni_count;
+                                }
+                            }
+                            s->d_uni.ensure(4 * s->uni_bits.size());
+                            HIPCHK(hipMemcpyAsync(s->d_uni.p, s->uni_bits.data(), 4 * s->uni_bits.size(),
+                                                  hipMemcpyHostToDevice, c->stream));
+                            s->uni_K = K;
+                        }
+                        if (s->uni_count) {
+                            uni = s->d_uni.as<uint32_t>();
+                            s->uni_given = s->uni_count;
+                        }
+                    }
                     kt.begin(3, c->stream);
                     HIPCHK(launch_la_stream_res(c->dt, dp, dx, dcr, P, rgeo, L0, c->clists.as<uint64_t>(),
                                                 (uint32_t)lwords, (uint32_t)rcw, c->npart.as<uint4>(),
                                                 c->normi.as<NormInfo>(), c->nstat.as<uint32_t>(),
                                                 c->nfall.as<unsigned long long>(), on, ok,
-                                                st, c->resctl.p, sel, rdiag, rsh, c->stream));
+                                                st, c->resctl.p, sel, rdiag, rsh, c->stream, uni));
                     kt.end(3, c->stream);
                     if (rdiag) {
                         uint64_t h[128] = {0};
@@ -1702,6 +1732,11 @@
                         if (h[36] + h[37] + h[38])
                             fprintf(stderr, "QS_RES_DIAG B3 -> B1 busy (ns per window, without the B1 wait): D %.0f, A %.0f, "
                                             "C %.0f\n", h[38] * 10.0 / nw, h[37] * 10.0 / nw, h[36] * 10.0 / nw);
+                        if (h[41])
+                            fprintf(stderr, "QS_RES_DIAG uniform windows %llu: %.2f us each from B1 to the window end, "
+                                            "%.2f rounds each; the other windows %.2f us each, boundaries included\n",
+                                    (unsigned long long)h[41], h[40] * 0.01 / (double)h[41], (double)h[42] / (double)h[41],
+                                    h[3] > h[41] ? (h[1] - h[40]) * 0.01 / (double)(h[3] - h[41]) : 0.0);
                         if (h[33])
                             fprintf(stderr, "QS_RES_DIAG last list of a window published %.2f us after the start of "
                                             "the window before it (%llu windows; after 13 us %llu, after 15 us %llu)\n",
@@ -2042,4 +2077,11 @@
     });
 }
 
-}
+qs_status qs_stream_uniform_windows(qs_ctx *c, qs_stream *s, uint32_t *windows) {
+    return guarded(c, [&] {
+        if (!s || !windows) fail(QS_EINVAL, "null stream or output");
+        *windows = s->ran ? s->uni_given : 0u;
+    });
+}
+
+}
diff --git a/custom-k8s-scheduler_amd/csrc/qs_kernels.hip b/custom-k8s-scheduler_amd/csrc/qs_kernels.hip
--- a/custom-k8s-scheduler_amd/csrc/qs_kernels.hip
+++ b/custom-k8s-scheduler_amd/csrc/qs_kernels.hip
@@ -201,11 +201,17 @@
     return (uint32_t)std::max(0, safe) * cus;
 }
 
+bool la_stream_res_takes_uniform(const LaGeom &geo, uint32_t feat, uint32_t W) {
+    return geo.k32 && W == 1 && geo.K <= 32 && res_uniform_class(feat, geo.E);
+}
+
 hipError_t launch_la_stream_res(const DevTable &t, const void *pods, const DPodX *podx, const DevCfg &c, uint32_t P,
                                 const LaGeom &geo, uint64_t *lists0, uint64_t *clists0, uint32_t lwords,
                                 uint32_t cwords, uint4 *npart, NormInfo *norm, uint32_t *stat, unsigned long long *nfall,
                                 int32_t *on, uint64_t *ok, uint64_t *st, void *ctl, uint32_t sel_blocks, uint64_t *rdiag,
-                                const ResShard &rsh, hipStream_t stream) {
+                                const ResShard &rsh0, hipStream_t stream, const uint32_t *uni) {
+    ResShard rsh = rsh0;
+    rsh.uni = la_stream_res_takes_uniform(geo, c.feat, rsh0.W) ? uni : nullptr;
     if (geo.G == 0 || (uint64_t)t.n * (t.wrows ? sizeof(DRowW) : sizeof(DRow)) >= (1ull << 31))
         return hipErrorInvalidValue;
     if (c.feat & kFeatStrat)
diff --git a/custom-k8s-scheduler_amd/csrc/qs_kernels.hpp b/custom-k8s-scheduler_amd/csrc/qs_kernels.hpp
--- a/custom-k8s-scheduler_amd/csrc/qs_kernels.hpp
+++ b/custom-k8s-scheduler_amd/csrc/qs_kernels.hpp
@@ -2213,6 +2213,11 @@
 
 constexpr uint32_t kResNormK = 32;
 constexpr uint32_t kResRing = 4;
+constexpr uint32_t kResUniR = 6;
+constexpr uint32_t kResUniMaxE = 5;
+constexpr bool res_uniform_class(uint32_t feat, uint32_t E) {
+    return (feat & (kFeatNorm | kFeatStrat)) == 0 && E <= kResUniMaxE;
+}
 constexpr uint32_t kResTStride = 65;
 constexpr size_t kResLdsMax = 96 * 1024;
 constexpr uint32_t kResSgprMax = 112;
@@ -2322,14 +2327,15 @@
     return ks;
 }
 
-template <uint32_t F, bool K32>
+template <uint32_t F, bool K32, bool UNI = false>
 __device__ __forceinline__ void la_resolve4_stream(uint32_t *lds, const DevTable &t, const PodT<F> *__restrict__ pods,
                                                    const DevCfg &c, uint32_t P, uint32_t K, uint32_t nwin,
                                                    const uint64_t *lists0, uint32_t lwords,
                                                    int32_t *__restrict__ out_node, uint64_t *__restrict__ out_key,
                                                    uint64_t *__restrict__ stamps, ResCtl *ctl, uint64_t *rdiag,
                                                    const DPodX *__restrict__ podx, const NormInfo *norm0,
-                                                   const uint32_t *stat0, unsigned long long *nfall) {
+                                                   const uint32_t *stat0, unsigned long long *nfall,
+                                                   const uint32_t *__restrict__ uni) {
     constexpr bool NORM = (F & kFeatNorm) != 0;
     constexpr bool R32 = K32 && !NORM;
     using KT = typename std::conditional<R32, uint32_t, uint64_t>::type;
@@ -2385,6 +2391,31 @@
     RowT<F>(*ringR)[64] = (RowT<F>(*)[64])rbase; rbase += kResRing * 64 * sizeof(RowT<F>);
     int4(*ringX)[64] = (int4(*)[64])rbase; rbase += kResRing * 64 * sizeof(int4);
     uint32_t *late = (uint32_t *)rbase;
+    constexpr uint32_t UR = kResUniR;
+    static_assert(UR >= 2 && UR % 2 == 0, "waves A and B write half of a slot ladder each");
+    static_assert(UR * 10 <= 64, "wave D packs a ladder's rungs (tv < 2^10, qs_key32.hpp) into 64 bits");
+    static_assert(32 * (sizeof(RowT<F>) + 16) + 2 * UR * 256 + 3 * 256 + 16 <= 2 * 64 * (sizeof(RowT<F>) + 16),
+                  "the uniform-window arrays fit in stage / stagex");
+    char *ubase = (char *)stage;
+    RowT<F> *unewR = (RowT<F> *)ubase; ubase += 32 * sizeof(RowT<F>);
+    int4 *unewX = (int4 *)ubase; ubase += 32 * sizeof(int4);
+    uint32_t(*uladS)[64] = (uint32_t(*)[64])ubase; ubase += UR * 256;
+    uint32_t(*uladC)[64] = (uint32_t(*)[64])ubase; ubase += UR * 256;
+    uint32_t *udS = (uint32_t *)ubase; ubase += 256;
+    uint32_t *udC = (uint32_t *)ubase; ubase += 256;
+    uint32_t *utmp = (uint32_t *)ubase; ubase += 256;
+    uint32_t *unext = (uint32_t *)ubase;
+    uint32_t *unew = unext + 1;
+    constexpr bool R32U = R32 && UNI;
+    auto uniw = [&](uint32_t w) -> bool { return R32U && uni && ((uni[w >> 5] >> (w & 31)) & 1u) != 0u; };
+    auto uni_follow = [&](uint32_t kend) {
+        do {
+            __syncthreads();
+            __syncthreads();
+        } while (*unext < kend);
+    };
+    (void)unewR; (void)unewX; (void)uladS; (void)uladC; (void)udS; (void)udC; (void)utmp; (void)unew;
+    (void)uniw; (void)uni_follow;
     const ResPub none{0, 0xFFFFFFFFu, -1, -1, 0, {0, 0}};
     ResPub32 *pub32 = (ResPub32 *)pub;
     const ResPub32 none32{0u, -1, -1, 0u};
@@ -2393,6 +2424,8 @@
     asm volatile("" : "+v"(cv.yd_both), "+v"(cv.yd_c), "+v"(cv.yd_m), "+v"(cv.wc), "+v"(cv.wm));
     uint64_t ts_ = 0, busy_ = 0, steps_ = 0, sub_[3] = {0, 0, 0};
     uint64_t bseg_[6] = {0, 0, 0, 0, 0, 0}, bt_ = 0;
+    uint64_t utime_ = 0;
+    uint32_t uwin_ = 0, urounds_ = 0;
     auto bmark = [&](int k) {
         if (rdiag) {
             const uint64_t t_ = __builtin_amdgcn_s_memrealtime();
@@ -2441,12 +2474,89 @@
             uint64_t res_key = 0, res_stamp = 0;
             ResPub pv = none;
             bool stopped = false;
+            const bool uw = uniw(w);
             if (NORM) __syncthreads();
             if (w > 0) bmark(5);
             __syncthreads();
             if (w > 0) bmark(3);
             if (rdiag && lane == 0) store_coh_u64(&rdiag[15], __builtin_amdgcn_s_memrealtime());
-            for (uint32_t i = 0; i < kend; ++i) {
+            if constexpr (R32U) {
+                if (uw) {
+                    const uint64_t tu0 = rdiag ? __builtin_amdgcn_s_memrealtime() : 0ull;
+                    const uint32_t clow = C1[1][lane] & kK32NodeMask;
+                    uint32_t i = 0, cct = 0;
+                    while (i < kend) {
+                        __syncthreads();
+                        uint64_t sl = 0, cl = 0;
+#pragma unroll
+                        for (uint32_t k = 0; k < UR; ++k) {
+                            sl |= (uint64_t)uladS[k][lane] << (10 * k);
+                            cl |= (uint64_t)uladC[k][lane] << (10 * k);
+                        }
+                        uint32_t ls = UR, lc = UR, ds = 0, dc = 0;
+                        for (;;) {
+                            const uint32_t st = (uint32_t)sl & 1023u, ct = (uint32_t)cl & 1023u;
+                            const uint32_t sk = st ? (k32_score(st) | dlow) : 0u;
+                            const uint32_t ck = ct ? (k32_score(ct) | clow) : 0u;
+                            const uint32_t m = wave_max_u32_dpp(sk > ck ? sk : ck);
+                            if (m == 0u) {
+                                if ((uint32_t)lane >= i) {
+                                    res_k32 = 0u;
+                                    if (stamps) res_stamp = __builtin_amdgcn_s_memrealtime();
+                                }
+                                i = kend;
+                                break;
+                            }
+                            if ((uint32_t)lane == i) {
+                                res_k32 = m;
+                                if (stamps) res_stamp = __builtin_amdgcn_s_memrealtime();
+                            }
+                            ++i;
+                            const uint64_t own_s = __ballot(sk == m);
+                            uint32_t left;
+                            if (own_s) {
+                                const int ol = (int)__builtin_ctzll(own_s);
+                                if (lane == ol) {
+                                    sl >>= 10;
+                                    --ls;
+                                    ++ds;
+                                }
+                                left = (uint32_t)__builtin_amdgcn_readlane((int)ls, ol);
+                            } else {
+                                const int ol = (int)__builtin_ctzll(__ballot(ck == m));
+                                if (lane == ol) {
+                                    cl >>= 10;
+                                    --lc;
+                                    ++dc;
+                                }
+                                left = (uint32_t)__builtin_amdgcn_readlane((int)lc, ol);
+                            }
+                            if (left == 0u || i >= kend) break;
+                        }
+                        udS[lane] = ds;
+                        udC[lane] = dc;
+                        if (lane == 0) *unext = i;
+                        won |= ds > 0u;
+                        cct += dc;
+                        ++urounds_;
+                        __syncthreads();
+                    }
+                    const uint64_t nm = __ballot(cct > 0u);
+                    if (cct > 0u) utmp[nd + (uint32_t)__popcll(nm & ((1ull << lane) - 1ull))] = clow;
+                    __builtin_amdgcn_wave_barrier();
+                    const uint32_t nnew = (uint32_t)__popcll(nm);
+                    if ((uint32_t)lane >= nd && (uint32_t)lane < nd + nnew) {
+                        dlow = utmp[lane];
+                        won = true;
+                    }
+                    nd += nnew;
+                    if (rdiag) {
+                        utime_ += __builtin_amdgcn_s_memrealtime() - tu0;
+                        ++uwin_;
+                    }
+                }
+            }
+            for (uint32_t i = 0, ke = uw ? 0u : kend; i < ke; ++i) {
                 if constexpr (R32) {
                     QS_RSTAMP_BEGIN()
                     const int par = i & 1, pp = par ^ 1;
@@ -2720,14 +2830,45 @@
                 return r;
             };
             if (NORM) __syncthreads();
-            if (wv == 1 && nd > 0)
+            bool uw = false;
+            if constexpr (R32U) uw = uniw(w);
+            if (wv == 1 && nd > 0 && !uw)
                 keyA[1][lane] = slot_key(S, SX, wp[0], podn(0), NORM ? Tcur[lane] : 0u);
             if (w > 0) bmark(0);
             __syncthreads();
             const uint32_t isig = 0;
+            if constexpr (R32U) {
+                if (uw) {
+                    const PodT<F> p0 = wp[0];
+                    if (wv == 1 && pend) {
+                        drain_stores();
+                        if (lane == 0) __hip_atomic_store((gu32 *)&ctl->done, pend, __ATOMIC_RELAXED, __HIP_MEMORY_SCOPE_AGENT);
+                        pend = 0;
+                    }
+                    constexpr uint32_t H = UR / 2;
+                    const uint32_t k0 = wv == 2 ? H : 0u;
+                    const bool act = (uint32_t)lane < nd;
+                    for (;;) {
+                        RowT<F> r = S;
+                        RowX x = SX;
+                        reserve_n(r, x, p0, (int)k0);
+#pragma unroll
+                        for (uint32_t k = 0; k < H; ++k) {
+                            const bool f = feasible<F>(r, x, p0, px);
+                            const uint32_t tot = fit_bal_total<F, FA>(r, x, p0, cv);
+                            uladS[k0 + k][lane] = (act && f) ? tot + 1 : 0u;
+                            reserve(r, x, p0, +1);
+                        }
+                        __syncthreads();
+                        __syncthreads();
+                        reserve_n(S, SX, p0, (int)udS[lane]);
+                        if (*unext >= kend) break;
+                    }
+                }
+            }
             PodT<F> pprev = wp[0], pcur = wp[0];
             PodN pnx = podn(1);
-            for (uint32_t i = 0; i < kend; ++i) {
+            for (uint32_t i = 0, ke = uw ? 0u : kend; i < ke; ++i) {
                 QS_RSTAMP_BEGIN()
                 const int par = i & 1, pp = par ^ 1;
                 ResPub pv = rpub(pp);
@@ -2765,8 +2906,21 @@
                 __syncthreads();
             }
             if (NORM && rpub((kend - 1) & 1).slot == -2) rescan_ab(kend - 1, w & 1);
-            apply(rpub((kend - 1) & 1), (kend - 1) & 1, pprev, s0 + kend - 1);
+            if (!uw) apply(rpub((kend - 1) & 1), (kend - 1) & 1, pprev, s0 + kend - 1);
             __syncthreads();
+            if constexpr (R32U) {
+                if (uw) {
+                    const uint32_t nn = *unew;
+                    if ((uint32_t)lane >= nd && (uint32_t)lane < nd + nn) {
+                        S = unewR[(uint32_t)lane - nd];
+                        if (F & kFeatExt) {
+                            const int4 e = unewX[(uint32_t)lane - nd];
+                            SX.ae0 = e.x; SX.re0 = e.y; SX.ae1 = e.z; SX.re1 = e.w;
+                        }
+                    }
+                    nd += nn;
+                }
+            }
             const uint32_t rk = xrank[lane];
             const bool keep = (uint32_t)lane < nd && rk != 0xFFFFFFFFu;
             if (wv == 1 && keep) {
@@ -3036,10 +3190,49 @@
             const KT e0 = ringE[s0 % kResRing][lane];
             c1 = (e0 != 0 && !dirty_bit(e0)) ? e0 : (KT)0;
             C1[1][lane] = c1;
+            const bool uw = uniw(w);
             if (w > 0) bmark(0);
             __syncthreads();
+            if constexpr (R32U) {
+                if (uw) {
+                    const PodT<F> p0 = wp[0];
+                    const RowT<F> r0 = ringR[s0 % kResRing][lane];
+                    RowX x0{};
+                    if (F & kFeatExt) {
+                        const int4 e = ringX[s0 % kResRing][lane];
+                        x0.ae0 = e.x; x0.re0 = e.y; x0.ae1 = e.z; x0.re1 = e.w;
+                    }
+                    uint32_t ct = 0;
+                    for (;;) {
+                        RowT<F> r = r0;
+                        RowX x = x0;
+                        reserve_n(r, x, p0, (int)ct);
+#pragma unroll
+                        for (uint32_t k = 0; k < UR; ++k) {
+                            const bool f = feasible<F>(r, x, p0, px);
+                            const uint32_t tot = fit_bal_total<F, FA>(r, x, p0, cv);
+                            uladC[k][lane] = (c1 != 0 && f) ? tot + 1 : 0u;
+                            reserve(r, x, p0, +1);
+                        }
+                        __syncthreads();
+                        __syncthreads();
+                        ct += udC[lane];
+                        if (*unext >= kend) break;
+                    }
+                    const uint64_t nm = __ballot(ct > 0u);
+                    if (ct > 0u) {
+                        const uint32_t rk = (uint32_t)__popcll(nm & ((1ull << lane) - 1ull));
+                        RowT<F> r = r0;
+                        RowX x = x0;
+                        reserve_n(r, x, p0, (int)ct);
+                        unewR[rk] = r;
+                        if (F & kFeatExt) unewX[rk] = make_int4(x.ae0, x.re0, x.ae1, x.re1);
+                    }
+                    if (lane == 0) *unew = (uint32_t)__popcll(nm);
+                }
+            }
             PodT<F> pcur = wp[0];
-            for (uint32_t i = 0; i < kend; ++i) {
+            for (uint32_t i = 0, ke = uw ? 0u : kend; i < ke; ++i) {
                 QS_RSTAMP_BEGIN()
                 const uint32_t g = s0 + i;
                 const int par = i & 1;
@@ -3099,8 +3292,13 @@
             const uint32_t ic = pfw ? kend - 3 : kend - 1;
             bool lt = hasnext;
             uint32_t rdyv = 0;
+            const bool uw = uniw(w);
             __syncthreads();
-            for (uint32_t i = 0; i < kend; ++i) {
+            if (uw) {
+                uni_follow(kend);
+                if (lane == 0) *late = 1u;
+            }
+            for (uint32_t i = 0, ke = uw ? 0u : kend; i < ke; ++i) {
                 const uint32_t g = s0 + i;
                 if (!(skip && i == 0)) ringE[(g + 2) % kResRing][lane] = kconv(ein);
                 if (i == ic) {
@@ -3128,8 +3326,10 @@
             const uint32_t s0 = w * K, kend = min(K, P - s0);
             const bool hasnext = w + 1 < nwin;
             const bool pfw = hasnext && kend >= 6;
+            const bool uw = uniw(w);
             __syncthreads();
-            for (uint32_t i = 0; i < kend; ++i) {
+            if (uw) uni_follow(kend);
+            for (uint32_t i = 0, ke = uw ? 0u : kend; i < ke; ++i) {
                 const uint32_t g = s0 + i;
                 const bool go = i + 1 < kend || (pfw ? *late == 0u : !hasnext);
                 if (go) {
@@ -3261,6 +3461,17 @@
             ndi = (uint32_t)__popcll(__ballot(xrank[lane] != 0xFFFFFFFFu));
             __syncthreads();
         }
+    } else {
+        for (uint32_t w = 0; w < nwin; ++w) {
+            const uint32_t kend = min(K, P - w * K);
+            const bool uw = uniw(w);
+            __syncthreads();
+            if (uw) uni_follow(kend);
+            else
+                for (uint32_t i = 0; i < kend; ++i) __syncthreads();
+            __syncthreads();
+            __syncthreads();
+        }
     }
     if (kResDiag && rdiag && lane == 0 && wv < 4) {
         rdiag[8 + wv] = busy_;
@@ -3272,12 +3483,13 @@
     if (rdiag && lane == 0 && wv == 0)
         for (int k = 0; k < 5; ++k) rdiag[27 + k] = bseg_[k];
     if (rdiag && lane == 0 && wv == 0) rdiag[38] = bseg_[5];
+    if (rdiag && lane == 0 && wv == 0) { rdiag[40] = utime_; rdiag[41] = uwin_; rdiag[42] = urounds_; }
     if (rdiag && lane == 0 && (wv == 1 || wv == 3)) rdiag[wv == 1 ? 37 : 36] = bseg_[0];
 }
 #undef QS_RSTAMP_BEGIN
 #undef QS_RSTAMP_END
 
-template <uint32_t F, int E, int E2, bool K32>
+template <uint32_t F, int E, int E2, bool K32, bool UNI = false>
 __global__ __launch_bounds__(kResBS) void k_la_stream_res(DevTable t, const PodT<F> *__restrict__ pods, DevCfg c,
                                                        uint32_t P, uint32_t K, uint32_t G, uint32_t L,
                                                        uint32_t chunk, uint32_t nwin, uint64_t *lists0,
@@ -3298,15 +3510,15 @@
             __hip_atomic_store(reinterpret_cast<uint64_t *>(rsh.peers[r] + rsh.hello) + rsh.rank, rsh.seq,
                                __ATOMIC_RELEASE, __HIP_MEMORY_SCOPE_SYSTEM);
     extern __shared__ __attribute__((aligned(16))) uint32_t lds[];
-    if ((F & kFeatNorm) == 0 && threadIdx.x >= 384) {
+    if (!UNI && (F & kFeatNorm) == 0 && threadIdx.x >= 384) {
         __syncthreads();
         for (uint32_t w = 0; w < nwin; ++w)
             for (uint32_t j = 0, nb = min(K, P - w * K) + 3; j < nb; ++j) __syncthreads();
         return;
     }
     const uint64_t t0 = rdiag ? __builtin_amdgcn_s_memrealtime() : 0ull;
-    la_resolve4_stream<F, K32>(lds, t, pods, c, P, K, nwin, lists0, lwords, out_node, out_key, stamps, ctl, rdiag,
-                               podx, norm0, stat0, nfall);
+    la_resolve4_stream<F, K32, UNI>(lds, t, pods, c, P, K, nwin, lists0, lwords, out_node, out_key, stamps, ctl, rdiag,
+                               podx, norm0, stat0, nfall, rsh.uni);
     if (rdiag && threadIdx.x == 0) { rdiag[1] = __builtin_amdgcn_s_memrealtime() - t0; rdiag[3] = nwin; }
 }
 
@@ -3334,6 +3546,15 @@
     ResCtl *rc = (ResCtl *)ctl;
 #define QS_RESK(EE, EE2, KK)                                                                                          \
     do {                                                                                                              \
+    if constexpr (KK && res_uniform_class(F, EE)) {                                                                  \
+        if (rsh.uni) {                                                                                                \
+            if (hipError_t ea = res_lds_attr((const void *)k_la_stream_res<F, EE, EE2, true, true>, lds4); ea != hipSuccess) return ea; \
+            hipLaunchKernelGGL((k_la_stream_res<F, EE, EE2, true, true>), grid, dim3(kResBS), lds4, stream, t, pp, c, P, K, G, L, \
+                               geo.chunk, nwin, lists0, clists0, lwords, cwords, on, ok, st, rc, rdiag, podx, npart0, norm0, \
+                               stat0, nfall, rsh);                                                                    \
+            break;                                                                                                    \
+        }                                                                                                             \
+    }                                                                                                                 \
     if (hipError_t ea = res_lds_attr((const void *)k_la_stream_res<F, EE, EE2, KK>, lds4); ea != hipSuccess) return ea; \
     hipLaunchKernelGGL((k_la_stream_res<F, EE, EE2, KK>), grid, dim3(kResBS), lds4, stream, t, pp, c, P, K, G, L,       \
                        geo.chunk, nwin, lists0, clists0, lwords, cwords, on, ok, st, rc, rdiag, podx, npart0, norm0,   \
@@ -3360,22 +3581,36 @@
 static int la_stream_res_per_cu(const LaGeom &geo, uint32_t n) {
     const size_t lds4 = res_stream_lds_bytes<F>(n, geo.k32 != 0);
     const void *fn = nullptr;
-#define QS_RESP(EE, KK) \
-    if (geo.E == EE && geo.e2 == 1 && (geo.k32 != 0) == KK) fn = (const void *)k_la_stream_res<F, EE, 1, KK>;
+    const void *fnu = nullptr;
+#define QS_RESPK(EE, EE2, KK) \
+    if (geo.E == EE && geo.e2 == EE2 && (geo.k32 != 0) == KK) { \
+        fn = (const void *)k_la_stream_res<F, EE, EE2, KK>; \
+        if constexpr (KK && res_uniform_class(F, EE)) fnu = (const void *)k_la_stream_res<F, EE, EE2, true, true>; \
+    }
+#define QS_RESP(EE, KK) QS_RESPK(EE, 1, KK)
     QS_RESP(3, true) QS_RESP(3, false) QS_RESP(5, true) QS_RESP(5, false) QS_RESP(7, true) QS_RESP(7, false)
     QS_RESP(8, true) QS_RESP(8, false) QS_RESP(16, true) QS_RESP(16, false)
 #undef QS_RESP
     if constexpr ((F & kFeatNorm) == 0) {
-#define QS_RESP2(EE, KK) \
-        if (geo.E == EE && geo.e2 == 2 && (geo.k32 != 0) == KK) fn = (const void *)k_la_stream_res<F, EE, 2, KK>;
+#define QS_RESP2(EE, KK) QS_RESPK(EE, 2, KK)
         QS_RESP2(5, true) QS_RESP2(5, false) QS_RESP2(7, true) QS_RESP2(7, false) QS_RESP2(8, true) QS_RESP2(8, false) QS_RESP2(16, true) QS_RESP2(16, false)
 #undef QS_RESP2
     }
+#undef QS_RESPK
     int per = 0;
     if (!fn || res_lds_attr(fn, lds4) != hipSuccess ||
         hipOccupancyMaxActiveBlocksPerMultiprocessor(&per, fn, kResBS, lds4) != hipSuccess) {
         (void)hipGetLastError();
         return 0;
+    }
+    if (fnu) {
+        int peru = 0;
+        if (res_lds_attr(fnu, lds4) != hipSuccess ||
+            hipOccupancyMaxActiveBlocksPerMultiprocessor(&peru, fnu, kResBS, lds4) != hipSuccess) {
+            (void)hipGetLastError();
+            return 0;
+        }
+        per = peru < per ? peru : per;
     }
     return per;
 }
diff --git a/custom-k8s-scheduler_amd/csrc/qs_launch.hpp b/custom-k8s-scheduler_amd/csrc/qs_launch.hpp
--- a/custom-k8s-scheduler_amd/csrc/qs_launch.hpp
+++ b/custom-k8s-scheduler_amd/csrc/qs_launch.hpp
@@ -73,12 +73,14 @@
     char *const *peers;
     uint64_t hello, flags, lists;
     uint64_t nflags, norm;
+    const uint32_t *uni;
 };
+bool la_stream_res_takes_uniform(const LaGeom &geo, uint32_t feat, uint32_t W);
 hipError_t launch_la_stream_res(const DevTable &t, const void *pods, const DPodX *podx, const DevCfg &c, uint32_t P,
                                 const LaGeom &geo, uint64_t *lists0, uint64_t *clists0, uint32_t lwords,
                                 uint32_t cwords, uint4 *npart, NormInfo *norm, uint32_t *stat, unsigned long long *nfall, int32_t *on,
                                 uint64_t *ok, uint64_t *st, void *ctl, uint32_t sel_blocks, uint64_t *rdiag,
-                                const ResShard &rsh, hipStream_t stream);
+                                const ResShard &rsh, hipStream_t stream, const uint32_t *uni = nullptr);
 
 hipError_t launch_la_window(const DevTable &t, const void *pods, const DPodX *podx, uint32_t s0,
                             uint32_t P, const DevCfg &c, const LaGeom &geo, const LaBufs &bufs,
diff --git a/custom-k8s-scheduler_amd/qsched/__init__.py b/custom-k8s-scheduler_amd/qsched/__init__.py
--- a/custom-k8s-scheduler_amd/qsched/__init__.py
+++ b/custom-k8s-scheduler_amd/qsched/__init__.py
@@ -283,6 +283,9 @@
         st = QsStats()
         self.s._chk(self.s.lib.qs_stream_run(self.s.ctx, self.h, MODES[mode], ctypes.byref(st)))
         self.stats = st.as_dict()
+        uw = ctypes.c_uint32(0)
+        self.s._chk(self.s.lib.qs_stream_uniform_windows(self.s.ctx, self.h, ctypes.byref(uw)))
+        self.stats["uniform_windows"] = int(uw.value)
         return self.stats
 
     def results(self):
diff --git a/custom-k8s-scheduler_amd/qsched/_abi.py b/custom-k8s-scheduler_amd/qsched/_abi.py
--- a/custom-k8s-scheduler_amd/qsched/_abi.py
+++ b/custom-k8s-scheduler_amd/qsched/_abi.py
@@ -156,6 +156,7 @@
     "qs_stream_run": (ctypes.c_int, [_P, _P, ctypes.c_int, _P]),
     "qs_stream_results": (ctypes.c_int, [_P, _P, _P, _P]),
     "qs_stream_stamps": (ctypes.c_int, [_P, _P, _P]),
+    "qs_stream_uniform_windows": (ctypes.c_int, [_P, _P, _P]),
     "qs_stream_fit_errors": (ctypes.c_int, [_P, _P, _P, ctypes.c_uint32, _P]),
     "qs_stream_fit_taints": (ctypes.c_int, [_P, _P, _P, ctypes.c_uint32, _P, _P]),
     "qs_stream_free": (ctypes.c_int, [_P, _P]),
diff --git a/include/qsched.h b/include/qsched.h
--- a/include/qsched.h
+++ b/include/qsched.h
@@ -189,6 +189,7 @@
 QS_API qs_status qs_stream_results(qs_ctx *ctx, qs_stream *s, int32_t *placement_p, uint64_t *best_key_p);
 QS_API qs_status qs_stream_free(qs_ctx *ctx, qs_stream *s);
 QS_API qs_status qs_stream_stamps(qs_ctx *ctx, qs_stream *s, uint64_t *stamps_p);
+QS_API qs_status qs_stream_uniform_windows(qs_ctx *ctx, qs_stream *s, uint32_t *windows);
 typedef enum qs_fit_reason {
     QS_FIT_TOO_MANY_PODS = 0,
     QS_FIT_CPU = 1,
```

New measurement: 2.291 million pods/s, median of 6. 3.4% higher.
